# simplify23/TPS_PP

Hardware: NVIDIA B200
Metric: tps_pp_rectified_img_per_s (higher is better)
Workload: dtype f32

## Files before the change

### include/tpspp.h

```cpp
#ifndef TPSPP_H_
#define TPSPP_H_

#include <stddef.h>
#include <stdint.h>

#ifdef __cplusplus
extern "C" {
#endif

#define TPSPP_ABI_VERSION 2

#if defined(__GNUC__)
#define TPSPP_API __attribute__((visibility("default")))
#else
#define TPSPP_API
#endif

typedef struct CUstream_st* tpspp_stream_t;

enum {
  TPSPP_OK = 0,
  TPSPP_E_INVALID = -1,
  TPSPP_E_CUDA = -2,
  TPSPP_E_UNSUPPORTED = -3,
  TPSPP_E_NO_DEVICE = -4
};

enum { TPSPP_F32 = 0, TPSPP_BF16 = 1, TPSPP_SRC0_BF16 = 2 };

enum {
  TPSPP_MODE_ATTENTION = 0,
  TPSPP_MODE_CLASSICAL = 1
};

enum {
  TPSPP_VARIANT_AUTO = 0,
  TPSPP_VARIANT_GENERIC = 1,
  TPSPP_VARIANT_STAGED = 2,
  TPSPP_VARIANT_TILED = 3
};

typedef struct tpspp_warp_cfg {
  int32_t batch;
  int32_t channels0;
  int32_t src0_h, src0_w;
  int32_t channels1;
  int32_t src1_h, src1_w;
  int32_t out_h, out_w;
  int32_t num_fiducial;
  int32_t mode;
  float theta;
  int32_t feat_dtype;
  int32_t variant;
} tpspp_warp_cfg;

TPSPP_API int tpspp_version(void);
TPSPP_API const char* tpspp_last_error(void);

TPSPP_API int tpspp_device_info(int* sm_count, int* cc_major, int* cc_minor);

TPSPP_API int tpspp_launch_profile(int enable);
TPSPP_API int tpspp_launch_profile_read(float* ms, int capacity, int* count);

TPSPP_API size_t tpspp_warp_workspace_bytes(const tpspp_warp_cfg* cfg);

TPSPP_API size_t tpspp_warp_fwd_workspace_bytes(const tpspp_warp_cfg* cfg);

TPSPP_API int tpspp_warp_fwd(const tpspp_warp_cfg* cfg, const void* src0, const void* src1,
                   const float* c_prime, const float* pc_score, const float* P_hat,
                   const float* P, const float* inv_delta_C, void* out0, void* out1,
                   float* grid_out, void* workspace, tpspp_stream_t stream);

TPSPP_API int tpspp_sample_fwd(const tpspp_warp_cfg* cfg, const void* src0, const void* src1,
                     const float* grid, void* out0, void* out1, tpspp_stream_t stream);

TPSPP_API int tpspp_warp_bwd(const tpspp_warp_cfg* cfg, const void* src0, const void* src1,
                   const float* c_prime, const float* pc_score, const float* P_hat,
                   const float* P, const float* inv_delta_C, const void* gout0,
                   const void* gout1, void* gsrc0, void* gsrc1, float* g_c_prime,
                   float* g_pc_score, void* workspace, tpspp_stream_t stream);

enum {
  TPSPP_HEAD_FP32 = 0,
  TPSPP_HEAD_TC = 1,
  TPSPP_HEAD_BF16 = 2
};

typedef struct tpspp_head_cfg {
  int32_t batch;
  int32_t height, width;
  int32_t point_h, point_w;
  int32_t p_stride;
  int32_t precision;
  int32_t flags;
} tpspp_head_cfg;

enum { TPSPP_HEAD_FLAG_WEIGHTS_CACHED = 1, TPSPP_HEAD_FLAG_UNFUSED_DOWN = 2, TPSPP_HEAD_FLAG_UNFUSED_SCORE = 4,
       TPSPP_HEAD_FLAG_TF32X3_CONV = 8, TPSPP_HEAD_FLAG_FEATGRID_BF16 = 16 };

enum {
  TPSPP_P_ENC0_W = 0, TPSPP_P_ENC0_B, TPSPP_P_ENC1_W, TPSPP_P_ENC1_B, TPSPP_P_ENC2_W, TPSPP_P_ENC2_B,
  TPSPP_P_ENC3_W, TPSPP_P_ENC3_B, TPSPP_P_CBAM_MLP0_W, TPSPP_P_CBAM_MLP2_W, TPSPP_P_CBAM_SP_W,
  TPSPP_P_CBAM_SP_B, TPSPP_P_DEC0_W, TPSPP_P_DEC0_B, TPSPP_P_DEC1_W, TPSPP_P_DEC1_B, TPSPP_P_DEC2_W,
  TPSPP_P_DEC2_B, TPSPP_P_DEC3_W, TPSPP_P_DEC3_B, TPSPP_P_PLIN0_W, TPSPP_P_PLIN0_B, TPSPP_P_PLIN1_W,
  TPSPP_P_PLIN1_B, TPSPP_P_FLIN0_W, TPSPP_P_FLIN0_B, TPSPP_P_FLIN1_W, TPSPP_P_FLIN1_B,
  TPSPP_P_NORM1_W, TPSPP_P_NORM1_B, TPSPP_P_MLP_H_W, TPSPP_P_MLP_W_W, TPSPP_P_PROJ_W, TPSPP_P_PROJ_B,
  TPSPP_P_NORM2_W, TPSPP_P_NORM2_B, TPSPP_P_FC1_W, TPSPP_P_FC1_B, TPSPP_P_FC2_W, TPSPP_P_FC2_B,
  TPSPP_P_LOC1A_W, TPSPP_P_LOC1A_B, TPSPP_P_LOC1B_W, TPSPP_P_LOC1B_B, TPSPP_P_LOC2_W, TPSPP_P_LOC2_B,
  TPSPP_P_DOWN0_W, TPSPP_P_DOWN0_B, TPSPP_P_DOWN1_W, TPSPP_P_DOWN1_B, TPSPP_P_DOWN2_W, TPSPP_P_DOWN2_B,
  TPSPP_P_DOWN0_1_W, TPSPP_P_DOWN0_1_B, TPSPP_P_DOWN1_1_W, TPSPP_P_DOWN1_1_B, TPSPP_P_DOWNFEAT_W,
  TPSPP_P_DOWNFEAT_B, TPSPP_P_COUNT
};

enum {
  TPSPP_WS_F0 = 0, TPSPP_WS_F1, TPSPP_WS_F2, TPSPP_WS_A0, TPSPP_WS_A1, TPSPP_WS_E0, TPSPP_WS_E1,
  TPSPP_WS_E2, TPSPP_WS_E3 , TPSPP_WS_CBAM, TPSPP_WS_D0, TPSPP_WS_D1, TPSPP_WS_D2,
  TPSPP_WS_DE , TPSPP_WS_X1, TPSPP_WS_V, TPSPP_WS_DE2 ,
  TPSPP_WS_P1 ,
  TPSPP_WS_WPREP , TPSPP_WS_T1, TPSPP_WS_FS ,
  TPSPP_WS_HID , TPSPP_WS_P1IMG , TPSPP_WS_COUNT
};

TPSPP_API size_t tpspp_head_workspace_bytes(const tpspp_head_cfg* cfg);
TPSPP_API int tpspp_head_workspace_offsets(const tpspp_head_cfg* cfg, size_t* offsets);

TPSPP_API int tpspp_head_fwd(const tpspp_head_cfg* cfg, const float* x, const float* o0, const float* o1,
                             const float* const* params, float* feat_grid, float* c_prime,
                             float* pc_score, void* workspace, tpspp_stream_t stream);

typedef struct {
  int32_t batch;
  int32_t height, width;
  int32_t precision;
  int32_t flags;
} tpspp_stage_cfg;

enum {
  TPSPP_SP_CONV1_W = 0, TPSPP_SP_CONV1_B, TPSPP_SP_BN1_W, TPSPP_SP_BN1_B, TPSPP_SP_BN1_MEAN, TPSPP_SP_BN1_VAR,
  TPSPP_SP_LAYER1 = 6,
  TPSPP_SP_LAYER2 = 36,
  TPSPP_SP_COUNT = 81
};

TPSPP_API size_t tpspp_stage_workspace_bytes(const tpspp_stage_cfg* cfg);
TPSPP_API int tpspp_stage_fwd(const tpspp_stage_cfg* cfg, const float* img, const float* const* params, float* o0, float* o1,
                              float* x, void* workspace, tpspp_stream_t stream);

typedef struct {
  int32_t batch, channels;
  int32_t height, width;
  int32_t num_fiducial;
  int32_t flags;
} tpspp_locnet_cfg;
enum { TPSPP_LP_FC1_W = 20, TPSPP_LP_FC1_B, TPSPP_LP_FC2_W, TPSPP_LP_FC2_B, TPSPP_LP_COUNT = 24 };
TPSPP_API size_t tpspp_locnet_workspace_bytes(const tpspp_locnet_cfg* cfg);
TPSPP_API int tpspp_locnet_fwd(const tpspp_locnet_cfg* cfg, const float* img, const float* const* params, float* c_prime,
                               void* workspace, tpspp_stream_t stream);

typedef struct {
  int32_t batch, cin;
  int32_t height, width;
  int32_t ksize;
  int32_t stride_h, stride_w;
  int32_t relu;
  int32_t nsrc;
  int32_t up_h[3], up_w[3];
} tpspp_conv_cfg;
TPSPP_API size_t tpspp_conv_workspace_bytes(const tpspp_conv_cfg* cfg);
TPSPP_API int tpspp_conv_fwd(const tpspp_conv_cfg* cfg, const float* x, const float* w, const float* bias, float* y,
                             void* workspace, tpspp_stream_t stream);
TPSPP_API int tpspp_conv_bwd(const tpspp_conv_cfg* cfg, const float* x, const float* w, const float* y, const float* gy,
                             float* gx, float* gw, float* gb, void* workspace, tpspp_stream_t stream);

typedef struct {
  int64_t rows;
  int32_t in_features, out_features;
  int32_t weight_batches;
  int32_t flags;
} tpspp_linear_cfg;
enum { TPSPP_LINEAR_FLAG_WEIGHTS_CACHED = 1 };
TPSPP_API size_t tpspp_linear_workspace_bytes(const tpspp_linear_cfg* cfg);
// ... 54 lines not shown
```

### tps_pp_b200/_native.py

```python
from __future__ import annotations

import ctypes
import os
from ctypes import POINTER, Structure, c_char_p, c_float, c_int, c_int32, c_size_t, c_void_p

_HERE = os.path.dirname(os.path.abspath(__file__))
LIB_PATH = os.environ.get("TPSPP_LIB", os.path.join(_HERE, "libtpspp.so"))

OK = 0
F32, BF16, SRC0_BF16 = 0, 1, 2
MODE_ATTENTION, MODE_CLASSICAL = 0, 1
VARIANT_AUTO, VARIANT_GENERIC, VARIANT_STAGED, VARIANT_TILED = 0, 1, 2, 3


class WarpCfg(Structure):
    _fields_ = [
        ("batch", c_int32), ("channels0", c_int32), ("src0_h", c_int32), ("src0_w", c_int32),
        ("channels1", c_int32), ("src1_h", c_int32), ("src1_w", c_int32),
        ("out_h", c_int32), ("out_w", c_int32), ("num_fiducial", c_int32), ("mode", c_int32),
        ("theta", c_float), ("feat_dtype", c_int32), ("variant", c_int32),
    ]


class HeadCfg(Structure):
    _fields_ = [
        ("batch", c_int32), ("height", c_int32), ("width", c_int32), ("point_h", c_int32), ("point_w", c_int32),
        ("p_stride", c_int32), ("precision", c_int32), ("flags", c_int32),
    ]


class StageCfg(Structure):
    _fields_ = [("batch", c_int32), ("height", c_int32), ("width", c_int32), ("precision", c_int32), ("flags", c_int32)]


class ConvCfg(Structure):
    _fields_ = [("batch", c_int32), ("cin", c_int32), ("height", c_int32), ("width", c_int32), ("ksize", c_int32),
                ("stride_h", c_int32), ("stride_w", c_int32), ("relu", c_int32), ("nsrc", c_int32),
                ("up_h", c_int32 * 3), ("up_w", c_int32 * 3)]


class LocnetCfg(Structure):
    _fields_ = [("batch", c_int32), ("channels", c_int32), ("height", c_int32), ("width", c_int32), ("num_fiducial", c_int32),
                ("flags", c_int32)]


LP_COUNT = 24


class AttnCfg(Structure):
    _fields_ = [("batch", c_int32), ("heads", c_int32), ("head_dim", c_int32), ("kv_len", c_int32), ("kv_capacity", c_int32),
                ("temperature", c_float), ("q_stride", c_int32), ("new_stride", c_int32), ("kv_head_major", c_int32)]


class AttnEncodeCfg(Structure):
    _fields_ = [("batch", c_int32), ("heads", c_int32), ("head_dim", c_int32), ("seq_len", c_int32), ("temperature", c_float),
                ("row_stride", c_int32)]


class OcrPrepCfg(Structure):
    _fields_ = [("n", c_int32), ("out_h", c_int32), ("out_w", c_int32), ("mean", c_float * 3), ("std", c_float * 3),
                ("pad_value", c_int32), ("flags", c_int32), ("packed_bytes", ctypes.c_int64)]


class LinearCfg(Structure):
    _fields_ = [("rows", ctypes.c_int64), ("in_features", c_int32), ("out_features", c_int32), ("weight_batches", c_int32),
                ("flags", c_int32)]


SP_COUNT = 81
HEAD_FP32, HEAD_TC, HEAD_BF16 = 0, 1, 2
HEAD_FLAG_WEIGHTS_CACHED = 1
HEAD_FLAG_UNFUSED_DOWN = 2
HEAD_FLAG_UNFUSED_SCORE = 4
HEAD_FLAG_TF32X3_CONV = 8
HEAD_FLAG_FEATGRID_BF16 = 16
LINEAR_FLAG_WEIGHTS_CACHED = 1
ACT_NONE, ACT_GELU = 0, 1
ABI_VERSION = 2
P_COUNT = 58
WS_NAMES = ("f0", "f1", "f2", "a0", "a1", "e0", "e1", "e2", "e3", "cbam", "d0", "d1", "d2", "de", "x1", "v", "de2", "p1", "wprep", "t1", "fs", "hid", "p1img")

_SIGNATURES = {
    "tpspp_version": (c_int, []),
    "tpspp_last_error": (c_char_p, []),
    "tpspp_last_launch_count": (c_int, []),
    "tpspp_launch_profile": (c_int, [c_int]),
    "tpspp_launch_profile_read": (c_int, [POINTER(ctypes.c_float), c_int, POINTER(c_int)]),
    "tpspp_device_info": (c_int, [POINTER(c_int), POINTER(c_int), POINTER(c_int)]),
    "tpspp_warp_workspace_bytes": (c_size_t, [POINTER(WarpCfg)]),
    "tpspp_warp_fwd_workspace_bytes": (c_size_t, [POINTER(WarpCfg)]),
    "tpspp_warp_fwd": (c_int, [POINTER(WarpCfg)] + [c_void_p] * 12),
    "tpspp_sample_fwd": (c_int, [POINTER(WarpCfg)] + [c_void_p] * 6),
    "tpspp_warp_bwd": (c_int, [POINTER(WarpCfg)] + [c_void_p] * 15),
    "tpspp_head_workspace_bytes": (c_size_t, [POINTER(HeadCfg)]),
    "tpspp_head_workspace_offsets": (c_int, [POINTER(HeadCfg), POINTER(c_size_t)]),
    "tpspp_head_fwd": (c_int, [POINTER(HeadCfg), c_void_p, c_void_p, c_void_p, POINTER(c_void_p),
                               c_void_p, c_void_p, c_void_p, c_void_p, c_void_p]),
    "tpspp_conv_workspace_bytes": (c_size_t, [POINTER(ConvCfg)]),
    "tpspp_conv_fwd": (c_int, [POINTER(ConvCfg)] + [c_void_p] * 6),
    "tpspp_conv_bwd": (c_int, [POINTER(ConvCfg)] + [c_void_p] * 9),
    "tpspp_convcat_fwd": (c_int, [POINTER(ConvCfg), POINTER(c_void_p)] + [c_void_p] * 5),
    "tpspp_convcat_bwd": (c_int, [POINTER(ConvCfg), POINTER(c_void_p)] + [c_void_p] * 3 + [POINTER(c_void_p)] + [c_void_p] * 4),
    "tpspp_locnet_workspace_bytes": (c_size_t, [POINTER(LocnetCfg)]),
    "tpspp_locnet_fwd": (c_int, [POINTER(LocnetCfg), c_void_p, POINTER(c_void_p), c_void_p, c_void_p, c_void_p]),
    "tpspp_attn_decode": (c_int, [POINTER(AttnCfg)] + [c_void_p] * 8),
    "tpspp_attn_encode": (c_int, [POINTER(AttnEncodeCfg)] + [c_void_p] * 6),
    "tpspp_ocr_prep": (c_int, [POINTER(OcrPrepCfg)] + [c_void_p] * 4),
    "tpspp_linear_fwd_ex": (c_int, [POINTER(LinearCfg)] + [c_void_p] * 4 + [c_int32] + [c_void_p] * 3),
    "tpspp_linear_ln_fwd": (c_int, [POINTER(LinearCfg)] + [c_void_p] * 4 + [c_int32] + [c_void_p] * 3 + [ctypes.c_float] + [c_void_p] * 3),
    "tpspp_linear_workspace_bytes": (c_size_t, [POINTER(LinearCfg)]),
    "tpspp_linear_fwd": (c_int, [POINTER(LinearCfg)] + [c_void_p] * 6),
    "tpspp_linear_bwd": (c_int, [POINTER(LinearCfg)] + [c_void_p] * 8),
    "tpspp_stage_workspace_bytes": (c_size_t, [POINTER(StageCfg)]),
    "tpspp_stage_fwd": (c_int, [POINTER(StageCfg), c_void_p, POINTER(c_void_p), c_void_p, c_void_p, c_void_p, c_void_p,
                                c_void_p]),
}
_OPTIONAL = {}

_lib = None


def exported_symbols():
    return sorted(_SIGNATURES)


def lib() -> ctypes.CDLL:
    global _lib
    if _lib is None:
        if not os.path.exists(LIB_PATH):
            raise RuntimeError(
                f"libtpspp.so not found at {LIB_PATH}: build it with `python -m tps_pp_b200.build` "
                "(there is no CPU/PyTorch fallback for the TPS++ hot path)")
        handle = ctypes.CDLL(LIB_PATH)
        for name, (res, args) in {**_SIGNATURES, **_OPTIONAL}.items():
            try:
                fn = getattr(handle, name)
            except AttributeError:
                if name in _OPTIONAL:
                    continue
                raise RuntimeError(f"{LIB_PATH} does not export {name}; rebuild it")
            fn.restype = res
            fn.argtypes = args
        if handle.tpspp_version() != ABI_VERSION:
            raise RuntimeError("libtpspp ABI version mismatch; rebuild it")
        _lib = handle
    return _lib


def last_error() -> str:
    return lib().tpspp_last_error().decode("utf-8", "replace")


def check(rc: int, what: str) -> None:
    if rc != OK:
        raise RuntimeError(f"{what} failed (code {rc}): {last_error()}")


def last_launch_count() -> int:
# ... 8 lines not shown
```

### tps_pp_b200/backbone.py

```python
from __future__ import annotations

from typing import Optional, Sequence

import torch
import torch.nn as nn
import torch.nn.functional as F

from . import functional as TF
from .registry import BACKBONES


class BasicBlock(nn.Module):
    expansion = 1

    def __init__(self, inplanes, planes, stride=1, downsample=None):
        super().__init__()
        self.conv1 = nn.Conv2d(inplanes, planes, kernel_size=1, stride=1, bias=False)
        self.bn1 = nn.BatchNorm2d(planes)
        self.relu = nn.ReLU(inplace=True)
        self.conv2 = nn.Conv2d(planes, planes, kernel_size=3, stride=stride, padding=1, bias=False)
        self.bn2 = nn.BatchNorm2d(planes)
        self.downsample = downsample
        self.stride = stride

    def forward(self, x):
        out = self.relu(self.bn1(self.conv1(x)))
        out = self.bn2(self.conv2(out))
        identity = x if self.downsample is None else self.downsample(x)
        return self.relu(out + identity)


@BACKBONES.register_module()
class ResNetABI_v2_large(nn.Module):
    def __init__(self, in_channels=3, stem_channels=32, base_channels=32, arch_settings=[3, 4, 6, 6, 3],
                 strides=[2, 1, 2, 1, 1], p_strides=[2, 1, 2, 1, 1], out_indices=None, last_stage_pool=False,
                 init_cfg=[dict(type='Xavier', layer='Conv2d'), dict(type='Constant', val=1, layer='BatchNorm2d')]):
        super().__init__()
        assert isinstance(in_channels, int)
        assert isinstance(stem_channels, int)
        assert isinstance(arch_settings, list) and all(isinstance(v, int) for v in arch_settings)
        assert isinstance(strides, list) and all(isinstance(v, int) for v in strides)
        assert len(arch_settings) == len(strides)
        assert out_indices is None or isinstance(out_indices, (list, tuple))
        assert isinstance(last_stage_pool, bool)
        self.init_cfg = init_cfg
        self.out_indices = out_indices
        self.last_stage_pool = last_stage_pool
        self.arch_settings = list(arch_settings)
        self.strides = list(strides)
        self.in_channels, self.stem_channels, self.base_channels = in_channels, stem_channels, base_channels
        self.conv1 = nn.Conv2d(in_channels, stem_channels, kernel_size=3, stride=1, padding=1)
        self.bn1 = nn.BatchNorm2d(stem_channels)
        self.relu1 = nn.ReLU()
        self.res_layers = []
        inplanes, planes = stem_channels, base_channels
        for i, blocks in enumerate(arch_settings):
            stride = strides[i]
            downsample = None
            if stride != 1 or inplanes != planes:
                downsample = nn.Sequential(nn.Conv2d(inplanes, planes, 1, stride, bias=False), nn.BatchNorm2d(planes))
            layers = [BasicBlock(inplanes, planes, stride=stride, downsample=downsample)]
            layers += [BasicBlock(planes, planes) for _ in range(1, blocks)]
            name = f'layer{i + 1}'
            self.add_module(name, nn.Sequential(*layers))
            self.res_layers.append(name)
            inplanes = planes
            planes *= 2
        self.stage_impl = "auto"
        self._stage_ws = {}
        self._last_stage_native = None

    def init_weights(self):
        for m in self.modules():
            if isinstance(m, nn.Conv2d):
                nn.init.xavier_normal_(m.weight, gain=1)
                if m.bias is not None:
                    nn.init.constant_(m.bias, 0)
            elif isinstance(m, nn.BatchNorm2d):
                nn.init.constant_(m.weight, 1)
                nn.init.constant_(m.bias, 0)

    def _stage_native_ok(self, x) -> bool:
        if self.stage_impl == "library":
            return False
        ok = (x.is_cuda and x.dtype == torch.float32 and x.dim() == 4 and x.shape[1] == 3 and x.shape[3] == 128
              and x.shape[2] % 4 == 0 and not self.training and not torch.is_grad_enabled()
              and self.in_channels == 3 and self.stem_channels == 32 and self.base_channels == 32
              and self.arch_settings[:2] == [3, 4] and self.strides[:2] == [1, 2])
        if self.stage_impl == "native" and not ok:
            raise RuntimeError("tps_pp_b200: stage_impl='native' needs eval mode, torch.no_grad(), fp32 CUDA images "
                               "[B,3,4k,128] and the nrtr_tps++ geometry (arch_settings[:2]=[3,4], strides[:2]=[1,2])")
        return ok

    def stage_tensors(self):
        out = [self.conv1.weight, self.conv1.bias, self.bn1.weight, self.bn1.bias, self.bn1.running_mean, self.bn1.running_var]
        for layer in (self.layer1, self.layer2):
            for blk in layer:
                out += [blk.conv1.weight, blk.bn1.weight, blk.bn1.bias, blk.bn1.running_mean, blk.bn1.running_var,
                        blk.conv2.weight, blk.bn2.weight, blk.bn2.bias, blk.bn2.running_mean, blk.bn2.running_var]
                if blk.downsample is not None:
                    ds = blk.downsample
                    out += [ds[0].weight, ds[1].weight, ds[1].bias, ds[1].running_mean, ds[1].running_var]
        return out

    def stage(self, img: torch.Tensor):
        self._last_stage_native = self._stage_native_ok(img)
        if self._last_stage_native:
            tensors = self.stage_tensors()
            key = (img.device.index, torch.cuda.current_stream(img.device).cuda_stream)
            stamp = (img.shape[0], img.shape[2], tuple((t.data_ptr(), t._version) for t in tensors))
            ws, ws_stamp = self._stage_ws.get(key, (None, None))
            o0, o1, x, ws = TF.stage_forward(img, tensors, ws, weights_cached=(ws_stamp == stamp))
            if len(self._stage_ws) >= 8 and key not in self._stage_ws:
                self._stage_ws.clear()
            self._stage_ws[key] = (ws, stamp)
            return x, [o0, o1]
        if not img.is_cuda:
            raise RuntimeError("tps_pp_b200.ResNetABI_v2_large runs on CUDA tensors only; there is no CPU fallback")
        x = self.relu1(self.bn1(self.conv1(img)))
        outs = []
        for name in self.res_layers[:2]:
            outs.append(x)
            x = getattr(self, name)(x)
        return x, outs

    def forward(self, x, tpsnet=None, test=False, **kwargs):
        x, outs = self.stage(x)
        outputs = None
        for i, name in enumerate(self.res_layers):
            if i < 2:
                continue
            if i == 2 and tpsnet is not None:
                outputs = tpsnet(x, outs, **kwargs)
                if outputs.get('output', None) is not None:
                    x = outputs['output']
            outs.append(x)
            x = getattr(self, name)(x)
        return {'output': x, 'img_ref': outputs.get('output', None) if outputs is not None else None}

    def return_feature(self, x, tpsnet=None, test=False):
        x, outs = self.stage(x)
        if tpsnet is None:
            return x
        for name in self.res_layers[2:]:
            x = getattr(self, name)(x)
        return x
```

### tps_pp_b200/csrc/common.cuh

```cuda
#pragma once
#include <cuda_runtime.h>
#include <cuda_bf16.h>
#include <stdint.h>
#include <stdio.h>
#include <stdarg.h>

#include "../../include/tpspp.h"

#if defined(__CUDA_ARCH__) && (__CUDA_ARCH__ < 1000)
#error "libtpspp is written for sm_100a (B200) only"
#endif

namespace tpspp {

void set_error(const char* fmt, ...);
void count_launch(int n = 1);
void prof_begin(cudaStream_t st);
void reset_launch_count();
int sm_count();
bool pdl_on();
void pdl_scope(bool on);
template <typename... KArgs, typename... Args>
inline void launch_k(void (*kern)(KArgs...), dim3 grid, dim3 block, size_t smem, cudaStream_t st, Args&&... args) {
  cudaLaunchConfig_t cfg = {};
  cfg.gridDim = grid;
  cfg.blockDim = block;
  cfg.dynamicSmemBytes = smem;
  cfg.stream = st;
  cudaLaunchAttribute at[1];
  at[0].id = cudaLaunchAttributeProgrammaticStreamSerialization;
  at[0].val.programmaticStreamSerializationAllowed = 1;
  cfg.attrs = at;
  cfg.numAttrs = pdl_on() ? 1 : 0;
  if (cudaLaunchKernelEx(&cfg, kern, static_cast<KArgs>(args)...) != cudaSuccess && cfg.numAttrs != 0) {
    cudaGetLastError();
    cfg.numAttrs = 0;
    cudaLaunchKernelEx(&cfg, kern, static_cast<KArgs>(args)...);
  }
}
#ifdef __CUDACC__
__device__ __forceinline__ void pdl_wait() { asm volatile("griddepcontrol.wait;" ::: "memory"); }
__device__ __forceinline__ void pdl_trigger() { asm volatile("griddepcontrol.launch_dependents;" ::: "memory"); }
#endif

#define TPSPP_CHECK_CUDA(expr)                                                        \
  do {                                                                                \
    cudaError_t _e = (expr);                                                          \
    if (_e != cudaSuccess) {                                                          \
      tpspp::set_error("%s failed: %s (%s:%d)", #expr, cudaGetErrorString(_e),        \
                       __FILE__, __LINE__);                                           \
      return TPSPP_E_CUDA;                                                            \
    }                                                                                 \
  } while (0)

#define TPSPP_REQUIRE(cond, ...)                                                      \
  do {                                                                                \
    if (!(cond)) {                                                                    \
      tpspp::set_error(__VA_ARGS__);                                                  \
      return TPSPP_E_INVALID;                                                         \
    }                                                                                 \
  } while (0)

struct WarpParams {
  int B, C0, H0, W0, C1, H1, W1, n, F, K;
  int mode;
  float theta;
  const void* src0;
  const void* src1;
  const float* c_prime;
  const float* score;
  const float* P_hat;
  const float* P;
  const float* hatC;
  const float* grid_in;
  void* out0;
  void* out1;
  float* grid_out;
  const void* gout0;
  const void* gout1;
  void* gsrc0;
  void* gsrc1;
  double* T_ws;
  float* g_grid;
  float* g_c_prime;
  float* g_score;
};

int validate_cfg(const tpspp_warp_cfg* cfg);
void fill_params(const tpspp_warp_cfg* cfg, WarpParams* p);
int bwd_nsplit(const tpspp_warp_cfg* cfg);

#ifdef __CUDACC__

struct Taps {
  int off, dx, dy;
  float w[4];
};

template <typename CT>
__device__ __forceinline__ CT clip_coord(CT v, int size) {
  return fmin((CT)(size - 1), fmax(v, (CT)0));
}

template <typename CT>
__device__ __forceinline__ Taps make_taps(CT gx, CT gy, int W, int H) {
  CT ix = ((gx + (CT)1) / (CT)2) * (CT)(W - 1);
  CT iy = ((gy + (CT)1) / (CT)2) * (CT)(H - 1);
  ix = clip_coord<CT>(ix, W);
  iy = clip_coord<CT>(iy, H);
  CT x0f = floor(ix), y0f = floor(iy);
  int x0 = (int)x0f, y0 = (int)y0f;
  CT tx = ix - x0f, ty = iy - y0f;
  CT ux = (x0f + (CT)1) - ix, uy = (y0f + (CT)1) - iy;
  Taps t;
  t.off = y0 * W + x0;
  t.dx = (x0 + 1 < W) ? 1 : 0;
  t.dy = (y0 + 1 < H) ? W : 0;
  t.w[0] = (float)(ux * uy);
  t.w[1] = t.dx ? (float)(tx * uy) : 0.f;
  t.w[2] = t.dy ? (float)(ux * ty) : 0.f;
  t.w[3] = (t.dx && t.dy) ? (float)(tx * ty) : 0.f;
// ... 205 lines not shown
```

### tps_pp_b200/csrc/head.cu

```cuda
#include "head.cuh"

#include <string.h>

namespace tpspp {

constexpr int CV_TM = 128;
constexpr int CV_KC = 32;
constexpr int CV_WLD = 68;
constexpr int CV_SMEM = (2 * CV_KC * CV_TM + 2 * CV_KC * CV_WLD) * 4;

template <int KS>
__global__ void __launch_bounds__(256, 2) conv_ffma_kernel(ConvArgs a) {
  extern __shared__ __align__(16) float smem[];
  float* As = smem;
  float* Ws = smem + 2 * CV_KC * CV_TM;
  constexpr int TAPS = KS * KS;
  const int tid = threadIdx.x;
  const int HoWo = a.Ho * a.Wo;
  const long long Mtot = (long long)a.B * HoWo;
  const long long m_base = (long long)blockIdx.x * CV_TM;
  const int Ktot = a.Ctot * TAPS;
  const int nchunks = (Ktot + CV_KC - 1) / CV_KC;

  const int lp = tid & (CV_TM - 1), lk0 = tid >> 7;
// ... 720 lines not shown
    }
#pragma unroll
    for (int i = 0; i < 8; ++i) {
      const int px = p0 + (i < 4 ? tx * 4 + i : 64 + tx * 4 + (i - 4));
      if (px >= n) continue;
      float* o = a.score + ((size_t)b * n + px) * F;
      const int k = ty * 2;
      if (k < F) o[k] = tanhf(acc[i][0] * a.scale);
      if (k + 1 < F) o[k + 1] = tanhf(acc[i][1] * a.scale);
    }
  }
}

struct HeadDims {
  int B, h, w, H2, W2, F, py, px, ps;
  int h1, w1, h2, w2;
};

static int head_dims(const tpspp_head_cfg* c, HeadDims* d) {
  TPSPP_REQUIRE(c != nullptr, "head cfg is NULL");
  TPSPP_REQUIRE(c->batch >= 0, "batch must be >= 0");
  TPSPP_REQUIRE(c->width == 64, "TPS_PP head needs feature-map width 64 (DGAB linear layers act on the width axis; "
                                "reference DGAB.py:36,52 -- SURVEY F4), got %d", c->width);
  TPSPP_REQUIRE(c->height >= 8 && c->height <= DG_MAXH && c->height % 8 == 0, "height must be a multiple of 8 in [8,%d]", DG_MAXH);
  TPSPP_REQUIRE(c->p_stride == 1 || c->p_stride == 2, "p_stride must be 1 or 2");
  d->B = c->batch; d->h = c->height; d->w = c->width; d->H2 = 2 * c->height; d->W2 = 2 * c->width;
  d->ps = c->p_stride;
  d->h1 = d->h / 2; d->w1 = d->w / 2;
  d->h2 = d->h1 / d->ps; d->w2 = d->w1 / d->ps;
  d->py = d->h2 / 2; d->px = d->w2;
  d->F = d->py * d->px;
  TPSPP_REQUIRE(d->py == c->point_h && d->px == c->point_w,
                "point_size (%d,%d) must equal the MSFA encoder's output lattice (%d,%d) (SURVEY F4)", c->point_h,
                c->point_w, d->py, d->px);
  TPSPP_REQUIRE(d->F <= 32 && d->F % 2 == 0, "num_fiducial must be even and <= 32 for the score kernel (got %d)", d->F);
  TPSPP_REQUIRE(c->precision == TPSPP_HEAD_FP32 || c->precision == TPSPP_HEAD_TC || c->precision == TPSPP_HEAD_BF16,
                "unknown precision %d", c->precision);
  return TPSPP_OK;
}

struct ConvLayerDesc { int w_idx, Ctot, KS, N, NT; };
constexpr int kNumTcLayers = 18;
enum { TCL_FLIN0 = 14, TCL_FLIN1 = 15, TCL_FC1 = 16, TCL_FC2 = 17 };
static const ConvLayerDesc kConvLayers[kNumTcLayers] = {
    {TPSPP_P_DOWN0_W, 32, 1, 64, 64},   {TPSPP_P_DOWN1_W, 32, 1, 64, 64},    {TPSPP_P_DOWN2_W, 64, 1, 64, 64},
    {TPSPP_P_DOWN0_1_W, 64, 3, 64, 64}, {TPSPP_P_DOWN1_1_W, 64, 3, 64, 64},  {TPSPP_P_DOWNFEAT_W, 192, 1, 64, 64},
    {TPSPP_P_ENC0_W, 192, 3, 64, 64},   {TPSPP_P_ENC1_W, 64, 3, 64, 64},     {TPSPP_P_ENC2_W, 64, 3, 64, 64},
    {TPSPP_P_ENC3_W, 64, 3, 64, 64},    {TPSPP_P_DEC0_W, 64, 3, 64, 64},     {TPSPP_P_DEC1_W, 64, 3, 64, 64},
    {TPSPP_P_DEC2_W, 64, 3, 64, 64},    {TPSPP_P_DEC3_W, 64, 3, 64, 64},
    {TPSPP_P_FLIN0_W, 64, 1, 32, 32},   {TPSPP_P_FLIN1_W, 32, 1, 128, 64},   {TPSPP_P_FC1_W, 64, 1, 256, 64},
    {TPSPP_P_FC2_W, 256, 1, 64, 64}};
static size_t wprep_total_floats() {
  size_t t = 0;
  for (int i = 0; i < kNumTcLayers; ++i) t += conv_tc_wprep_floats(kConvLayers[i].Ctot, kConvLayers[i].KS, kConvLayers[i].N);
  return t;
}

static void head_offsets(const HeadDims& d, size_t* off, size_t* total) {
  const size_t B = d.B;
  size_t sz[TPSPP_WS_COUNT];
  const size_t big = B * 64 * d.H2 * d.W2, mid = B * 64 * d.h * d.w;
  sz[TPSPP_WS_F0] = big; sz[TPSPP_WS_F1] = big; sz[TPSPP_WS_F2] = mid; sz[TPSPP_WS_A0] = mid; sz[TPSPP_WS_A1] = mid;
  sz[TPSPP_WS_E0] = mid; sz[TPSPP_WS_E1] = B * 64 * d.h1 * d.w1; sz[TPSPP_WS_E2] = B * 64 * d.h2 * d.w2;
  sz[TPSPP_WS_E3] = B * 64 * d.F; sz[TPSPP_WS_CBAM] = B * 64 * d.F; sz[TPSPP_WS_D0] = sz[TPSPP_WS_E2];
  sz[TPSPP_WS_D1] = sz[TPSPP_WS_E1]; sz[TPSPP_WS_D2] = mid; sz[TPSPP_WS_DE] = mid; sz[TPSPP_WS_X1] = mid;
  sz[TPSPP_WS_V] = mid; sz[TPSPP_WS_DE2] = mid; sz[TPSPP_WS_P1] = B * d.F * 128;
  sz[TPSPP_WS_WPREP] = wprep_total_floats();
  sz[TPSPP_WS_T1] = B * d.h * d.w * 32;
  sz[TPSPP_WS_FS] = B * d.h * d.w * 128;
  sz[TPSPP_WS_HID] = mid * 4;
  sz[TPSPP_WS_P1IMG] = B * 8192;
  size_t cur = 0;
  for (int i = 0; i < TPSPP_WS_COUNT; ++i) {
    off[i] = cur;
    cur += (sz[i] * sizeof(float) + 255) / 256 * 256;
  }
  *total = cur + 256;
}

static ConvSrc mk_src(const float* p, int C, int H, int W, int nhwc, int uh = 1, int uw = 1, int bf16 = 0) {
  ConvSrc s; s.ptr = p; s.C = C; s.H = H; s.W = W; s.uh = uh; s.uw = uw; s.nhwc = nhwc; s.bf16 = bf16; return s;
}

static int run_conv(int KS, ConvSrc s0, ConvSrc s1, ConvSrc s2, const float* w, const float* bias, const float* skip,
                    float* out, int out_nhwc, int B, int Ho, int Wo, int sh, int sw, cudaStream_t st,
                    const float* wprep = nullptr, int mode = CM_TF32X3, int out_bf16 = 0, int skip_bf16 = 0) {
  ConvArgs a;
  a.out_nhwc = out_nhwc; a.out_bf16 = out_bf16; a.skip_bf16 = skip_bf16;
  a.act = CONV_ACT_RELU; a.act_scale = 1.f; a.Cout = 64; a.wimg_stride = 0; a.skip_pre = 0; a.out_cstride = 0; a.zi = 0;
  a.src[0] = s0; a.src[1] = s1; a.src[2] = s2;
  a.weight = w; a.bias = bias; a.skip = skip; a.out = out;
  a.B = B; a.Ho = Ho; a.Wo = Wo; a.Ctot = s0.C + s1.C + s2.C; a.sh = sh; a.sw = sw; a.pad = (KS == 3) ? 1 : 0;
  if (wprep != nullptr && conv_tc_eligible(a, KS)) return run_conv_tc(KS, a, wprep, 64, st, mode);
  const long long M = (long long)B * Ho * Wo;
  const unsigned grid = (unsigned)((M + CV_TM - 1) / CV_TM);
  if (KS == 1) conv_ffma_kernel<1><<<grid, 256, CV_SMEM, st>>>(a);
  else conv_ffma_kernel<3><<<grid, 256, CV_SMEM, st>>>(a);
  count_launch();
  TPSPP_CHECK_CUDA(cudaGetLastError());
  return TPSPP_OK;
}

static int head_attrs_once() {
  static thread_local int done_dev = -1;
  int dev = 0;
  TPSPP_CHECK_CUDA(cudaGetDevice(&dev));
  if (done_dev == dev) return TPSPP_OK;
  TPSPP_CHECK_CUDA(cudaFuncSetAttribute(conv_ffma_kernel<1>, cudaFuncAttributeMaxDynamicSharedMemorySize, CV_SMEM));
  TPSPP_CHECK_CUDA(cudaFuncSetAttribute(conv_ffma_kernel<3>, cudaFuncAttributeMaxDynamicSharedMemorySize, CV_SMEM));
  TPSPP_CHECK_CUDA(cudaFuncSetAttribute(dgab_mlp_kernel, cudaFuncAttributeMaxDynamicSharedMemorySize, ML_SMEM));
  TPSPP_CHECK_CUDA(cudaFuncSetAttribute(score_kernel, cudaFuncAttributeMaxDynamicSharedMemorySize, SC_SMEM));
  TPSPP_CHECK_CUDA(cudaFuncSetAttribute(loc_p1_kernel, cudaFuncAttributeMaxDynamicSharedMemorySize, 64 * 1024));
  done_dev = dev;
  return TPSPP_OK;
}

}

using namespace tpspp;

extern "C" size_t tpspp_head_workspace_bytes(const tpspp_head_cfg* cfg) {
  HeadDims d;
  if (head_dims(cfg, &d) != TPSPP_OK) return 0;
  size_t off[TPSPP_WS_COUNT], total;
  head_offsets(d, off, &total);
  return total;
}

extern "C" int tpspp_head_workspace_offsets(const tpspp_head_cfg* cfg, size_t* offsets) {
  HeadDims d;
  int rc = head_dims(cfg, &d);
  if (rc != TPSPP_OK) return rc;
  TPSPP_REQUIRE(offsets != nullptr, "offsets is NULL");
  size_t total;
  head_offsets(d, offsets, &total);
  return TPSPP_OK;
}

extern "C" int tpspp_head_fwd(const tpspp_head_cfg* cfg, const float* x, const float* o0, const float* o1,
                              const float* const* P, float* feat_grid, float* c_prime, float* pc_score,
                              void* workspace, tpspp_stream_t stream) {
  reset_launch_count();
  prof_begin((cudaStream_t)stream);
  HeadDims d;
  int rc = head_dims(cfg, &d);
  if (rc != TPSPP_OK) return rc;
  if (d.B == 0) return TPSPP_OK;
  TPSPP_REQUIRE(x && o0 && o1 && P && feat_grid && c_prime && pc_score && workspace, "tpspp_head_fwd: null pointer");
  TPSPP_REQUIRE(((uintptr_t)workspace & 255) == 0, "tpspp_head_fwd: workspace must be 256-byte aligned");
  for (int i = 0; i < TPSPP_P_COUNT; ++i) {
    TPSPP_REQUIRE(P[i] != nullptr, "tpspp_head_fwd: params[%d] is NULL", i);
    TPSPP_REQUIRE(((uintptr_t)P[i] & 15) == 0, "tpspp_head_fwd: params[%d] must be 16-byte aligned (vector loads)", i);
  }
  if (d.B == 0) return TPSPP_OK;
  rc = head_attrs_once();
  if (rc != TPSPP_OK) return rc;
  cudaStream_t st = (cudaStream_t)stream;
  struct PdlScope { PdlScope(bool on) { pdl_scope(on); } ~PdlScope() { pdl_scope(false); } } pdl_guard(cfg->precision != TPSPP_HEAD_FP32);
  size_t off[TPSPP_WS_COUNT], total;
  head_offsets(d, off, &total);
  auto W = [&](int i) { return reinterpret_cast<float*>((char*)workspace + off[i]); };
  const ConvSrc none = mk_src(nullptr, 0, 1, 1, 0);
  constexpr int NCHW = 0, NHWC = 1;
  const int B = d.B, h = d.h, w = d.w, H2 = d.H2, W2 = d.W2;

  const float* wp[kNumTcLayers];
  for (int i = 0; i < kNumTcLayers; ++i) wp[i] = nullptr;
  const bool bf16 = cfg->precision == TPSPP_HEAD_BF16;
  const bool tc = cfg->precision == TPSPP_HEAD_TC || bf16;
  const bool weights_cached = (cfg->flags & TPSPP_HEAD_FLAG_WEIGHTS_CACHED) != 0;
  int cmode[14];
  for (int i = 0; i < 14; ++i) {
    const bool one = kConvLayers[i].KS == 1;
    cmode[i] = (bf16 && !one) ? CM_BF16 : ((one || (cfg->flags & TPSPP_HEAD_FLAG_TF32X3_CONV)) ? CM_TF32X3 : CM_MIX);
  }
  if (tc) {
    WPrepLayer L[kNumTcLayers];
    float* cur = W(TPSPP_WS_WPREP);
    for (int i = 0; i < kNumTcLayers; ++i) {
      L[i].w = P[kConvLayers[i].w_idx]; L[i].out = cur; L[i].Ctot = kConvLayers[i].Ctot;
      L[i].taps = kConvLayers[i].KS * kConvLayers[i].KS; L[i].N = kConvLayers[i].N; L[i].NT = kConvLayers[i].NT; L[i].scale = nullptr; L[i].dg_cin = 0; L[i].dg_ci0 = 0;
      L[i].bf16 = i < 14 ? cmode[i] : CM_TF32X3;
      wp[i] = cur;
      cur += conv_tc_wprep_floats(kConvLayers[i].Ctot, kConvLayers[i].KS, kConvLayers[i].N);
    }
    if (!weights_cached) {
      rc = conv_tc_prepare_weights(L, kNumTcLayers, st);
      if (rc != TPSPP_OK) return rc;
    }
  }
#define RUN(...) do { rc = run_conv(__VA_ARGS__); if (rc != TPSPP_OK) return rc; } while (0)
  bool fused_down = false;
  if (tc && !(cfg->flags & TPSPP_HEAD_FLAG_UNFUSED_DOWN)) {
    rc = run_down_fused(x, o0, o1, wp[0], wp[1], wp[2], wp[5], P[TPSPP_P_DOWN0_B], P[TPSPP_P_DOWN1_B], P[TPSPP_P_DOWN2_B],
                        P[TPSPP_P_DOWNFEAT_B], W(TPSPP_WS_F0), W(TPSPP_WS_F1), W(TPSPP_WS_F2), feat_grid, B, h, w, st, bf16 ? 1 : 0,
                        (bf16 && (cfg->flags & TPSPP_HEAD_FLAG_FEATGRID_BF16)) ? 1 : 0);
    if (rc < 0) return rc;
    fused_down = rc == TPSPP_OK;
    TPSPP_REQUIRE(fused_down || !bf16, "head: the bf16 mode needs the fused down kernel's geometry (width 64, 16-byte aligned inputs)");
  }
  const int bs = (bf16 && fused_down) ? 1 : 0;
  if (!fused_down) {
  RUN(1, mk_src(o0, 32, H2, W2, NCHW), none, none, P[TPSPP_P_DOWN0_W], P[TPSPP_P_DOWN0_B], nullptr, W(TPSPP_WS_F0), NCHW, B, H2, W2, 1, 1, st, wp[0], cmode[0]);
  RUN(1, mk_src(o1, 32, H2, W2, NCHW), none, none, P[TPSPP_P_DOWN1_W], P[TPSPP_P_DOWN1_B], nullptr, W(TPSPP_WS_F1), NCHW, B, H2, W2, 1, 1, st, wp[1], cmode[1]);
  RUN(1, mk_src(x, 64, h, w, NCHW), none, none, P[TPSPP_P_DOWN2_W], P[TPSPP_P_DOWN2_B], nullptr, W(TPSPP_WS_F2), NCHW, B, h, w, 1, 1, st, wp[2], cmode[2]);
  }
  RUN(3, mk_src(W(TPSPP_WS_F0), 64, H2, W2, NCHW, 1, 1, bs), none, none, P[TPSPP_P_DOWN0_1_W], P[TPSPP_P_DOWN0_1_B], nullptr, W(TPSPP_WS_A0), NCHW, B, h, w, 2, 2, st, wp[3], cmode[3], bs);
  RUN(3, mk_src(W(TPSPP_WS_F1), 64, H2, W2, NCHW, 1, 1, bs), none, none, P[TPSPP_P_DOWN1_1_W], P[TPSPP_P_DOWN1_1_B], nullptr, W(TPSPP_WS_A1), NCHW, B, h, w, 2, 2, st, wp[4], cmode[4], bs);
  if (!fused_down)
  RUN(1, mk_src(W(TPSPP_WS_F0), 64, H2, W2, NCHW), mk_src(W(TPSPP_WS_F1), 64, H2, W2, NCHW), mk_src(W(TPSPP_WS_F2), 64, h, w, NCHW, 2, 2),
      P[TPSPP_P_DOWNFEAT_W], P[TPSPP_P_DOWNFEAT_B], nullptr, feat_grid, NCHW, B, H2, W2, 1, 1, st, wp[5], cmode[5]);
  RUN(3, mk_src(W(TPSPP_WS_A0), 64, h, w, NCHW, 1, 1, bs), mk_src(W(TPSPP_WS_A1), 64, h, w, NCHW, 1, 1, bs), mk_src(W(TPSPP_WS_F2), 64, h, w, NCHW, 1, 1, bs),
      P[TPSPP_P_ENC0_W], P[TPSPP_P_ENC0_B], nullptr, W(TPSPP_WS_E0), NCHW, B, h, w, 1, 1, st, wp[6], cmode[6], bs);
  RUN(3, mk_src(W(TPSPP_WS_E0), 64, h, w, NCHW, 1, 1, bs), none, none, P[TPSPP_P_ENC1_W], P[TPSPP_P_ENC1_B], nullptr, W(TPSPP_WS_E1), NCHW, B, d.h1, d.w1, 2, 2, st, wp[7], cmode[7]);
  RUN(3, mk_src(W(TPSPP_WS_E1), 64, d.h1, d.w1, NCHW), none, none, P[TPSPP_P_ENC2_W], P[TPSPP_P_ENC2_B], nullptr, W(TPSPP_WS_E2), NCHW, B, d.h2, d.w2, d.ps, d.ps, st, wp[8], cmode[8]);
  RUN(3, mk_src(W(TPSPP_WS_E2), 64, d.h2, d.w2, NCHW), none, none, P[TPSPP_P_ENC3_W], P[TPSPP_P_ENC3_B], nullptr, W(TPSPP_WS_E3), NCHW, B, d.py, d.px, 2, 1, st, wp[9], cmode[9]);
  launch_k(cbam_kernel, dim3(B), dim3(256), 0, st, (const float*)W(TPSPP_WS_E3), W(TPSPP_WS_CBAM), P[TPSPP_P_CBAM_MLP0_W], P[TPSPP_P_CBAM_MLP2_W],
           P[TPSPP_P_CBAM_SP_W], P[TPSPP_P_CBAM_SP_B], d.py, d.px);
  count_launch();
  TPSPP_CHECK_CUDA(cudaGetLastError());
  RUN(3, mk_src(W(TPSPP_WS_CBAM), 64, d.py, d.px, NCHW, 2, 1), none, none, P[TPSPP_P_DEC0_W], P[TPSPP_P_DEC0_B], W(TPSPP_WS_E2), W(TPSPP_WS_D0), NCHW, B, d.h2, d.w2, 1, 1, st, wp[10], cmode[10]);
  RUN(3, mk_src(W(TPSPP_WS_D0), 64, d.h2, d.w2, NCHW, d.ps, d.ps), none, none, P[TPSPP_P_DEC1_W], P[TPSPP_P_DEC1_B], W(TPSPP_WS_E1), W(TPSPP_WS_D1), NCHW, B, d.h1, d.w1, 1, 1, st, wp[11], cmode[11]);
  RUN(3, mk_src(W(TPSPP_WS_D1), 64, d.h1, d.w1, NCHW, 2, 2), none, none, P[TPSPP_P_DEC2_W], P[TPSPP_P_DEC2_B], W(TPSPP_WS_E0), W(TPSPP_WS_D2), NCHW, B, h, w, 1, 1, st, wp[12], cmode[12], bs, bs);
  RUN(3, mk_src(W(TPSPP_WS_D2), 64, h, w, NCHW, 1, 1, bs), none, none, P[TPSPP_P_DEC3_W], P[TPSPP_P_DEC3_B], nullptr, W(TPSPP_WS_DE), NCHW, B, h, w, 1, 1, st, wp[13], cmode[13]);
#undef RUN
  {
    LocArgs a;
    a.e3 = W(TPSPP_WS_E3);
    a.wa = P[TPSPP_P_LOC1A_W]; a.ba = P[TPSPP_P_LOC1A_B]; a.wb = P[TPSPP_P_LOC1B_W]; a.bb = P[TPSPP_P_LOC1B_B];
    a.wc = P[TPSPP_P_LOC2_W]; a.bc = P[TPSPP_P_LOC2_B];
    a.wp0 = P[TPSPP_P_PLIN0_W]; a.bp0 = P[TPSPP_P_PLIN0_B]; a.wp1 = P[TPSPP_P_PLIN1_W]; a.bp1 = P[TPSPP_P_PLIN1_B];
    a.c_prime = c_prime; a.p1 = W(TPSPP_WS_P1); a.F = d.F;
    a.p1img = (tc && d.F == 32) ? W(TPSPP_WS_P1IMG) : nullptr;
    const size_t smem = (size_t)(d.F * 65 + d.F * 256 + 2 * d.F + d.F * 33) * sizeof(float);
    launch_k(loc_p1_kernel, dim3(B), dim3(256), smem, st, a);
    count_launch();
    TPSPP_CHECK_CUDA(cudaGetLastError());
  }
  {
    DgabArgs a;
    a.x = W(TPSPP_WS_DE); a.e3 = W(TPSPP_WS_E3);
    a.n1w = P[TPSPP_P_NORM1_W]; a.n1b = P[TPSPP_P_NORM1_B]; a.n2w = P[TPSPP_P_NORM2_W]; a.n2b = P[TPSPP_P_NORM2_B];
    a.wh = P[TPSPP_P_MLP_H_W]; a.ww = P[TPSPP_P_MLP_W_W]; a.wp = P[TPSPP_P_PROJ_W]; a.bp = P[TPSPP_P_PROJ_B];
    a.x1 = W(TPSPP_WS_X1); a.v = W(TPSPP_WS_V); a.H = h; a.F = d.F;
    {
      TPSPP_REQUIRE((h == 8 || h == 16) && d.F <= 32 && dgab_warp_smem(h, d.F) <= 220 * 1024, "DGAB: unsupported geometry h=%d F=%d", h, d.F);
      const size_t smem = dgab_warp_smem(h, d.F);
      auto kern = h == 8 ? dgab_warp_kernel<8> : dgab_warp_kernel<16>;
      TPSPP_CHECK_CUDA(cudaFuncSetAttribute(kern, cudaFuncAttributeMaxDynamicSharedMemorySize, (int)smem));
      int grid = sm_count();
      if (grid > (B * 64 + DW_WARPS - 1) / DW_WARPS) grid = (B * 64 + DW_WARPS - 1) / DW_WARPS;
      launch_k(kern, dim3(grid), dim3(DW_WARPS * 32), smem, st, a, B * 64);
    }
    count_launch();
    TPSPP_CHECK_CUDA(cudaGetLastError());
    const long long R = (long long)B * 64 * h;
    if (tc) {
      rc = run_mlp_fused(W(TPSPP_WS_V), W(TPSPP_WS_X1), wp[TCL_FC1], P[TPSPP_P_FC1_B], wp[TCL_FC2], P[TPSPP_P_FC2_B],
                         W(TPSPP_WS_DE2), R, st);
      if (rc < 0) return rc;
      if (rc == 1) {
      ConvArgs g;
      memset(&g, 0, sizeof(g));
      g.src[0] = mk_src(W(TPSPP_WS_V), 64, 1, (int)R, NHWC); g.src[1] = none; g.src[2] = none;
      g.B = 1; g.Ho = 1; g.Wo = (int)R; g.Ctot = 64; g.sh = 1; g.sw = 1; g.pad = 0; g.out_nhwc = 1;
      g.bias = P[TPSPP_P_FC1_B]; g.skip = nullptr; g.out = W(TPSPP_WS_HID); g.act = CONV_ACT_GELU; g.act_scale = 1.f;
      g.Cout = 256; g.wimg_stride = 0; g.weight = nullptr;
      rc = run_conv_tc(1, g, wp[TCL_FC1], 64, st);
      if (rc != TPSPP_OK) return rc;
      g.src[0] = mk_src(W(TPSPP_WS_HID), 256, 1, (int)R, NHWC); g.Ctot = 256;
      g.bias = P[TPSPP_P_FC2_B]; g.skip = W(TPSPP_WS_X1); g.out = W(TPSPP_WS_DE2); g.act = CONV_ACT_NONE; g.Cout = 64;
      rc = run_conv_tc(1, g, wp[TCL_FC2], 64, st);
      if (rc != TPSPP_OK) return rc;
      }
// ... 50 lines not shown
```

### tps_pp_b200/csrc/head.cuh

```cuda
#pragma once
#include "common.cuh"

namespace tpspp {

struct ConvSrc {
  const float* ptr;
  int C, H, W, uh, uw;
  int nhwc;
  int bf16;
};
struct ConvArgs {
  ConvSrc src[3];
  const float* weight;
  const float* bias;
  const float* skip;
  float* out;
  int B, Ho, Wo, Ctot, sh, sw, pad;
  int out_nhwc;
  int act;
  float act_scale;
  int Cout;
  long long wimg_stride;
  int skip_pre;
  int out_cstride;
  int zi;
  int out_bf16, skip_bf16;
  int splitk;
};
enum { CONV_ACT_RELU = 0, CONV_ACT_NONE = 1, CONV_ACT_GELU = 2, CONV_ACT_TANH = 3 };
enum { CM_TF32X3 = 0, CM_BF16 = 1, CM_MIX = 2 };


bool conv_tc_eligible(const ConvArgs& a, int KS);
int run_conv_tc(int KS, const ConvArgs& a, const float* wprep, int NT, cudaStream_t st, int mode = CM_TF32X3);
int run_mlp_fused(const float* v, const float* x1, const float* w1img, const float* b1, const float* w2img, const float* b2,
                  float* out, long long R, cudaStream_t st);
int run_down_fused(const float* x, const float* o0, const float* o1, const float* w0img, const float* w1img, const float* w2img,
                   const float* wfimg, const float* b0, const float* b1, const float* b2, const float* bf, float* f0, float* f1,
                   float* f2, float* fg, int B, int h, int w, cudaStream_t st, int out_bf16 = 0, int fg_bf16 = 0);
int run_score_fused(const float* de2, const float* w0img, const float* w1img, const float* p1img, const float* b0, const float* b1,
                    float* score, int B, int h, int w, int F, float scale, cudaStream_t st);
size_t conv_tc_wprep_floats(int Ctot, int KS, int N);

struct WPrepLayer {
  const float* w;
  float* out;
  int Ctot, taps, N, NT;
  const float* scale;
  int dg_cin, dg_ci0;
  int bf16;
};
constexpr int WPREP_MAX_LAYERS = 20;
size_t wgrad_rows_ws_floats(long long R, int K, int N, int batches);
int run_wgrad_rows(const float* gy, const float* x, float* gw, float* gb, long long R, int K, int N, int batches, float* ws,
                   cudaStream_t st);
int conv_tc_prepare_weights(const WPrepLayer* layers, int nlayers, cudaStream_t st);

}
```

### tps_pp_b200/csrc/head_tc.cu

```cuda
#include "head.cuh"
#include "tc.cuh"

#include <cuda.h>
#include <string.h>

namespace tpspp {

constexpr int TC_TM = 128, TC_KC = 32;
constexpr int TC_A_LBO = TC_TM * 16 + 16;
constexpr int TC_A_BYTES = (TC_KC / 4) * TC_A_LBO;
__host__ __device__ constexpr int tc_b_bytes(int NT) { return NT * TC_KC * 4; }
__host__ __device__ constexpr int tc_stage_bytes(int NT) { return 2 * TC_A_BYTES + 2 * tc_b_bytes(NT); }
__host__ __device__ constexpr int tc_smem_bytes(int NT) { return 2 * tc_stage_bytes(NT) + 64 + TC_TM * 16; }
constexpr int TC_PRODUCERS = 256, TC_THREADS = TC_PRODUCERS + 32;
__host__ __device__ constexpr int tc_tmem_cols(int NT) { return NT == 64 ? 256 : 128; }

struct ConvTcArgs {
  ConvArgs c;
  const float* wprep;
};

__device__ __forceinline__ float tc_gelu(float x) { return 0.5f * x * (1.f + erff(x * 0.70710678118654752440f)); }
__device__ __forceinline__ float tc_gelu_fast(float x) {
  const float z = fabsf(x) * 0.70710678118654752440f;
// ... 161 lines not shown
      if (lane == 0) mbar_arrive(&fbars[buf]);
    };
    gather(va);
    if (nchunks > 1) gather(vb);
    for (int ch = 0; ch < nchunks; ch += 2) {
      produce(ch, va);
      if (ch + 1 < nchunks) produce(ch + 1, vb);
    }
    const int last = nchunks - 1;
    mbar_wait_bounded(&bars[last & 1], (uint32_t)((last >> 1) & 1));
    tc_fence_after();
  }
  if (warp < TC_PRODUCERS / 32) {
    const int wq = warp & 3, half = warp >> 2;
    const long long m = m_base + wq * 32 + lane;
    const int b = (m < Mtot) ? (int)(m / HoWo) : 0;
    const int rem = (m < Mtot) ? (int)(m - (long long)b * HoWo) : 0;
#pragma unroll 1
    for (int pass = 0; pass < HC / 16; ++pass) {
      float acc[16], part[16];
      const uint32_t taddr = tmem_d + ((uint32_t)(wq * 32) << 16) + (uint32_t)(half * HC + pass * 16);
      tmem_ld_cols<16>(taddr, acc);
      tmem_ld_cols<16>(taddr + 2 * NT, part);
#pragma unroll
      for (int j = 0; j < 16; ++j) acc[j] += part[j];
      if (nchunks > 1) {
        tmem_ld_cols<16>(taddr + NT, part);
#pragma unroll
        for (int j = 0; j < 16; ++j) acc[j] += part[j];
      }
      const int cb = co_off + half * HC + pass * 16;
      if (m < Mtot && a.out_nhwc) {
        const size_t o0 = (size_t)m * a.Cout + cb;
#pragma unroll
        for (int j = 0; j < 16; j += 4) {
          float4 bs = make_float4(0.f, 0.f, 0.f, 0.f);
          if (a.bias != nullptr) bs = __ldg(reinterpret_cast<const float4*>(a.bias + cb + j));
          float4 r = make_float4(tc_act(acc[j] + bs.x, a.act, a.act_scale), tc_act(acc[j + 1] + bs.y, a.act, a.act_scale),
                                 tc_act(acc[j + 2] + bs.z, a.act, a.act_scale), tc_act(acc[j + 3] + bs.w, a.act, a.act_scale));
          if (a.skip != nullptr) {
            const float4 sk = __ldg(reinterpret_cast<const float4*>(a.skip + o0 + j));
            r.x += sk.x; r.y += sk.y; r.z += sk.z; r.w += sk.w;
          }
          *reinterpret_cast<float4*>(a.out + o0 + j) = r;
        }
      } else if (m < Mtot) {
        const size_t o0 = ((size_t)b * a.Cout + cb) * HoWo + rem;
#pragma unroll
        for (int j = 0; j < 16; ++j) {
          float r = tc_act(acc[j] + (a.bias != nullptr ? __ldg(a.bias + cb + j) : 0.f), a.act, a.act_scale);
          const size_t o = o0 + (size_t)j * HoWo;
          if (a.skip != nullptr) r += __ldg(a.skip + o);
          a.out[o] = r;
        }
      }
    }
  }
  tc_fence_before();
  __syncthreads();
  if (warp == 0) tmem_dealloc(tmem_d, tc_tmem_cols(NT));
}


__host__ __device__ constexpr uint32_t mix_b_bf(int NT) { return (uint32_t)NT * 128u; }
__host__ __device__ constexpr uint32_t mix_b_lo(int NT) { return (uint32_t)NT * 192u; }
constexpr uint32_t MIX_B_BF = mix_b_bf(64), MIX_B_LO = mix_b_lo(64);

template <int NT>
__device__ __forceinline__ void mix_mma_chunk(uint32_t tmem_d, uint32_t a_base, uint32_t b_base, uint32_t idesc_tf, uint32_t idesc_bf,
                                              bool first) {
#pragma unroll
  for (int j = 0; j < TC_KC / 16; ++j) {
    const uint64_t dbw = umma_smem_desc(b_base + mix_b_bf(NT) + j * 2 * (NT * 16), NT * 16, 128);
    const uint64_t dbl = umma_smem_desc(b_base + mix_b_lo(NT) + j * 2 * (NT * 16), NT * 16, 128);
    umma_ts_f16(tmem_d + 64, a_base + 32 + j * 8, dbw, idesc_bf, (first && j == 0) ? 0u : 1u);
    umma_ts_f16(tmem_d + 64, a_base + 48 + j * 8, dbl, idesc_bf, 1u);
  }
#pragma unroll
  for (int j = 0; j < TC_KC / 8; ++j) {
    const uint64_t dbh = umma_smem_desc(b_base + j * 2 * (NT * 16), NT * 16, 128);
    umma_ts_tf32(tmem_d, a_base + j * 8, dbh, idesc_tf, (first && j == 0) ? 0u : 1u);
  }
}
template <int NT>
__device__ __forceinline__ void mix_mma_chunk_probed(uint32_t d, uint32_t a_base, uint64_t bdesc0, uint32_t idesc_tf, uint32_t idesc_bf,
                                                     uint32_t accumulate, uint32_t commit_bar, uint32_t next_a_bar, uint32_t next_w_bar,
                                                     uint32_t next_parity, uint32_t& ok_a, uint32_t& ok_w) {
  constexpr int KS2 = 2 * NT, BW0 = 8 * NT, BL0 = 12 * NT;
  asm volatile(
      "{\n"
      ".reg .pred pa, pw, pf, pt;\n"
      ".reg .b64 dsc;\n"
      ".reg .b32 ta, tc;\n"
      "mbarrier.test_wait.parity.shared::cta.b64 pa, [%2], %4;\n"
      "mbarrier.test_wait.parity.shared::cta.b64 pw, [%3], %4;\n"
      "setp.ne.b32 pf, %9, 0;\n"
      "setp.eq.u32 pt, %4, %4;\n"
      "add.u32 tc, %5, 64;\n"
      "add.u32 ta, %6, 32;\n add.u64 dsc, %7, %12;\n"
      "tcgen05.mma.cta_group::1.kind::f16 [tc], [ta], dsc, %11, pf;\n"
      "add.u32 ta, %6, 48;\n add.u64 dsc, %7, %13;\n"
      "tcgen05.mma.cta_group::1.kind::f16 [tc], [ta], dsc, %11, pt;\n"
      "add.u32 ta, %6, 40;\n add.u64 dsc, %7, %14;\n"
      "tcgen05.mma.cta_group::1.kind::f16 [tc], [ta], dsc, %11, pt;\n"
      "add.u32 ta, %6, 56;\n add.u64 dsc, %7, %15;\n"
      "tcgen05.mma.cta_group::1.kind::f16 [tc], [ta], dsc, %11, pt;\n"
      "tcgen05.mma.cta_group::1.kind::tf32 [%5], [%6], %7, %10, pf;\n"
      "add.u32 ta, %6, 8;\n add.u64 dsc, %7, %16;\n"
      "tcgen05.mma.cta_group::1.kind::tf32 [%5], [ta], dsc, %10, pt;\n"
      "add.u32 ta, %6, 16;\n add.u64 dsc, %7, %17;\n"
      "tcgen05.mma.cta_group::1.kind::tf32 [%5], [ta], dsc, %10, pt;\n"
      "add.u32 ta, %6, 24;\n add.u64 dsc, %7, %18;\n"
      "tcgen05.mma.cta_group::1.kind::tf32 [%5], [ta], dsc, %10, pt;\n"
      "tcgen05.commit.cta_group::1.mbarrier::arrive::one.shared::cluster.b64 [%8];\n"
      "selp.u32 %0, 1, 0, pa;\n"
      "selp.u32 %1, 1, 0, pw;\n"
      "}\n"
      : "=r"(ok_a), "=r"(ok_w)
      : "r"(next_a_bar), "r"(next_w_bar), "r"(next_parity), "r"(d), "r"(a_base), "l"(bdesc0), "r"(commit_bar), "r"(accumulate),
        "r"(idesc_tf), "r"(idesc_bf), "n"(BW0), "n"(BL0), "n"(BW0 + KS2), "n"(BL0 + KS2), "n"(KS2), "n"(2 * KS2), "n"(3 * KS2)
      : "memory");
}
__device__ __forceinline__ void mix_split(const float (&v)[16], float (&hi)[16], uint32_t (&lo2)[8], uint32_t (&a2)[8]) {
#pragma unroll
  for (int i = 0; i < 16; ++i) hi[i] = __uint_as_float(__float_as_uint(v[i]) & 0xFFFFE000u);
#pragma unroll
  for (int i = 0; i < 8; ++i) {
    const __nv_bfloat162 l2 = __floats2bfloat162_rn(v[2 * i] - hi[2 * i], v[2 * i + 1] - hi[2 * i + 1]);
    const __nv_bfloat162 x2 = __floats2bfloat162_rn(v[2 * i], v[2 * i + 1]);
    lo2[i] = *reinterpret_cast<const uint32_t*>(&l2);
    a2[i] = *reinterpret_cast<const uint32_t*>(&x2);
  }
}
__device__ __forceinline__ void mix_store_a(uint32_t stage_addr, int kh, const float (&v)[16]) {
  float hi[16];
  uint32_t lo2[8], a2[8];
#pragma unroll
  for (int i = 0; i < 16; ++i) hi[i] = __uint_as_float(__float_as_uint(v[i]) & 0xFFFFE000u);
#pragma unroll
  for (int i = 0; i < 8; ++i) {
    const __nv_bfloat162 l2 = __floats2bfloat162_rn(v[2 * i] - hi[2 * i], v[2 * i + 1] - hi[2 * i + 1]);
    const __nv_bfloat162 x2 = __floats2bfloat162_rn(v[2 * i], v[2 * i + 1]);
    lo2[i] = *reinterpret_cast<const uint32_t*>(&l2);
    a2[i] = *reinterpret_cast<const uint32_t*>(&x2);
  }
  tmem_st16(stage_addr + (uint32_t)(kh * 16), hi);
  tmem_st8(stage_addr + (uint32_t)(32 + kh * 8), lo2);
  tmem_st8(stage_addr + (uint32_t)(48 + kh * 8), a2);
}

template <int PLANE>
__device__ __forceinline__ void ts_load16(const float* q, float (&v)[16], bool ok) {
#pragma unroll
  for (int i = 0; i < 16; ++i) v[i] = ok ? __ldg(q + i * PLANE) : 0.f;
}

constexpr int TS_B_BYTES = tc_b_bytes(64);
constexpr int TS_STAGE = 2 * TS_B_BYTES;
constexpr int TS_SMEM = 2 * TS_STAGE + 64 + TC_TM * 16 + 256;

template <int KS, int MODE>
__global__ void __launch_bounds__(TC_THREADS, 2) conv_ts_kernel(ConvTcArgs t) {
  constexpr bool BF16 = MODE == CM_BF16, MIX = MODE == CM_MIX;
  constexpr int NT = 64;
  constexpr int W_BYTES = BF16 ? NT * TC_KC * 2 : 2 * TS_B_BYTES;
  constexpr int A_COL0 = BF16 ? 64 : 128;
  constexpr int A_STAGE = BF16 ? 16 : 64;
  constexpr int TMEM_COLS = BF16 ? 128 : 256;
  extern __shared__ __align__(1024) unsigned char smem[];
  uint64_t* bars = reinterpret_cast<uint64_t*>(smem + 2 * TS_STAGE);
  uint64_t* wbars = bars + 2;
  uint64_t* fbars = bars + 4;
  uint32_t* tmem_slot = reinterpret_cast<uint32_t*>(bars + 6);
  int4* geo = reinterpret_cast<int4*>(smem + 2 * TS_STAGE + 64);
  float* bias_s = reinterpret_cast<float*>(smem + 2 * TS_STAGE + 64 + TC_TM * 16);
  const ConvArgs& a = t.c;
  const int tid = threadIdx.x, lane = tid & 31;
  const int warp = __shfl_sync(0xffffffffu, tid >> 5, 0);

  if (tid == 0) {
    mbar_init(&bars[0], 1); mbar_init(&bars[1], 1);
    mbar_init(&wbars[0], 1); mbar_init(&wbars[1], 1);
    mbar_init(&fbars[0], TC_PRODUCERS / 32); mbar_init(&fbars[1], TC_PRODUCERS / 32);
    fence_barrier_init();
  }
  if (tid < NT) bias_s[tid] = (a.bias != nullptr && tid < a.Cout) ? __ldg(a.bias + tid) : 0.f;
  if (warp == 0) tmem_alloc(tmem_slot, TMEM_COLS);
  tc_fence_before();
  __syncthreads();
  tc_fence_after();
  const uint32_t tmem_d = *tmem_slot;
  pdl_trigger();
  pdl_wait();

  const int HoWo = a.Ho * a.Wo;
  const long long Mtot = (long long)a.B * HoWo;
  const long long m_base = (long long)blockIdx.x * TC_TM;
  const int Ctot = a.Ctot;
  const int nchunks = (Ctot * KS * KS) / TC_KC;
  const unsigned char* wimg = reinterpret_cast<const unsigned char*>(t.wprep);

  if (tid < TC_TM) {
    const long long lm = m_base + tid;
    int4 gq = make_int4(0, 0, 0, 0);
    if (lm < Mtot) {
// ... 125 lines not shown
      tc_fence_before();
      __syncwarp();
      if (lane == 0) mbar_arrive(&fbars[buf]);
    };
    gather(va);
    if (nchunks > 1) gather(vb);
    for (int ch = 0; ch < nchunks; ch += 2) {
      produce(ch, va);
      if (ch + 1 < nchunks) produce(ch + 1, vb);
    }
    const int last = nchunks - 1;
    mbar_wait_bounded(&bars[last & 1], (uint32_t)((last >> 1) & 1));
    tc_fence_after();

    const int wq = warp & 3, half = warp >> 2;
    const long long m = m_base + wq * 32 + lane;
    const int b = (m < Mtot) ? (int)(m / HoWo) : 0;
    const int rem = (m < Mtot) ? (int)(m - (long long)b * HoWo) : 0;
#pragma unroll 1
    for (int pass = 0; pass < 2; ++pass) {
      float acc[16], part[16];
      const uint32_t taddr = lane_addr + (uint32_t)(half * 32 + pass * 16);
      tmem_ld_cols<16>(taddr, acc);
      if (!BF16) {
        tmem_ld_cols<16>(taddr + 64, part);
#pragma unroll
        for (int j = 0; j < 16; ++j) acc[j] += part[j];
      }
      const int cb = half * 32 + pass * 16;
      if (m < Mtot && a.out_nhwc) {
        const size_t o0 = (size_t)m * a.Cout + cb;
#pragma unroll
        for (int j = 0; j < 16; j += 4) {
          float4 bs = make_float4(0.f, 0.f, 0.f, 0.f);
          if (a.bias != nullptr) bs = __ldg(reinterpret_cast<const float4*>(a.bias + cb + j));
          float4 r = make_float4(tc_act(acc[j] + bs.x, a.act, a.act_scale), tc_act(acc[j + 1] + bs.y, a.act, a.act_scale),
                                 tc_act(acc[j + 2] + bs.z, a.act, a.act_scale), tc_act(acc[j + 3] + bs.w, a.act, a.act_scale));
          if (a.skip != nullptr) {
            const float4 sk = __ldg(reinterpret_cast<const float4*>(a.skip + o0 + j));
            r.x += sk.x; r.y += sk.y; r.z += sk.z; r.w += sk.w;
          }
          *reinterpret_cast<float4*>(a.out + o0 + j) = r;
        }
      } else if (m < Mtot) {
        const float4* b4 = reinterpret_cast<const float4*>(bias_s + cb);
#pragma unroll
        for (int j = 0; j < 16; j += 4) {
          const float4 bs = b4[j >> 2];
          acc[j] += bs.x; acc[j + 1] += bs.y; acc[j + 2] += bs.z; acc[j + 3] += bs.w;
        }
        const size_t o0 = ((size_t)b * (a.out_cstride ? a.out_cstride : a.Cout) + cb) * HoWo + rem;
        if (cb >= a.Cout) continue;
        if (a.skip != nullptr && a.skip_pre) {
          const float* sk = a.skip + o0;
#pragma unroll
          for (int j = 0; j < 16; ++j) acc[j] += __ldg(sk + (size_t)j * HoWo);
        }
        if (a.act == CONV_ACT_RELU) {
#pragma unroll
          for (int j = 0; j < 16; ++j) acc[j] = fmaxf(acc[j], 0.f);
        } else {
#pragma unroll
          for (int j = 0; j < 16; ++j) acc[j] = tc_act(acc[j], a.act, a.act_scale);
        }
        if (a.skip != nullptr && !a.skip_pre) {
          const float* sk = a.skip + o0;
#pragma unroll
          for (int j = 0; j < 16; ++j) acc[j] += __ldg(sk + (size_t)j * HoWo);
        }
        float* po = a.out + o0;
#pragma unroll
        for (int j = 0; j < 16; ++j) po[(size_t)j * HoWo] = acc[j];
      }
    }
  }
  tc_fence_before();
  __syncthreads();
  if (warp == 0) tmem_dealloc(tmem_d, TMEM_COLS);
}

struct ConvTmaArgs {
  ConvTcArgs t;
  CUtensorMap tmap[3];
  int TW, TH, BW, BH;
  int TX, TPI;
  int S;
  int XH;
};
constexpr int TM_XH = 4;
constexpr int TM_TILE_MAX = 32 * (4 * 72) * 4;
constexpr int TM_TILE_BF = 17408;
__host__ __device__ constexpr int tm_tile_bytes(int KS) { return KS == 3 ? ((TM_TILE_MAX + 1023) / 1024) * 1024 : 16384; }
__host__ __device__ constexpr int tm_tile_bufs(int KS) { return KS == 3 ? 2 : 4; }
__host__ __device__ constexpr int tm_smem_bytes(int KS) { return tm_tile_bufs(KS) * tm_tile_bytes(KS) + 2 * TS_STAGE + (KS == 3 ? 4096 : 0) + 512 + 1024; }
constexpr int TM_THREADS = TC_THREADS + 32;

__device__ __forceinline__ void tma_load_4d(void* dst, const CUtensorMap* tm, int c0, int c1, int c2, int c3, uint64_t* bar,
                                            uint64_t policy) {
  asm volatile(
      "cp.async.bulk.tensor.4d.shared::cluster.global.mbarrier::complete_tx::bytes.L2::cache_hint "
      "[%0], [%1, {%3, %4, %5, %6}], [%2], %7;" ::"r"(smem_u32(dst)),
      "l"(reinterpret_cast<uint64_t>(tm)), "r"(smem_u32(bar)), "r"(c0), "r"(c1), "r"(c2), "r"(c3), "l"(policy)
      : "memory");
}

template <int KS, int MODE, int NT = 64>
__global__ void __launch_bounds__(TM_THREADS, 2) conv_tma_kernel(const __grid_constant__ ConvTmaArgs g) {
  constexpr bool BF16 = MODE == CM_BF16, MIX = MODE == CM_MIX;
  constexpr int T = KS * KS;
  static_assert(NT == 64 || NT == 32, "64 or 32 output channels per tile");
  const int XH = g.XH;
  const bool SBF = (BF16 && KS == 3) && g.t.c.src[0].bf16 != 0;
  const int ntb_rt = SBF ? 4 : tm_tile_bufs(KS);
  const int tile_stride = SBF ? TM_TILE_BF : tm_tile_bytes(KS);
  constexpr int CT = (BF16 && KS == 3) ? 3 : 1;
  constexpr int W_TAP = BF16 ? NT * TC_KC * 2 : 2 * tc_b_bytes(NT);
  constexpr int W_BYTES = CT * W_TAP;
  constexpr int NS = (BF16 && KS == 3) ? 3 : 2;
  constexpr int A_BASE = NS == 3 ? 64 : 128, A_STRIDE = NS == 3 ? 48 : 64;
  constexpr int WS_STRIDE = NS == 3 ? 12288 : TS_STAGE;
  constexpr int TILE_BYTES = tm_tile_bytes(KS);
  constexpr int NTB = tm_tile_bufs(KS);
  extern __shared__ unsigned char smem_raw[];
  unsigned char* smem = reinterpret_cast<unsigned char*>((reinterpret_cast<uintptr_t>(smem_raw) + 1023) & ~(uintptr_t)1023);
  unsigned char* tiles = smem;
  unsigned char* wst = smem + NTB * TILE_BYTES;
  uint64_t* bars = reinterpret_cast<uint64_t*>(wst + (NS == 3 ? 3 * 12288 : 2 * TS_STAGE));
  uint64_t* a_empty = bars;
  uint64_t* a_full = bars + 3;
  uint64_t* w_full = bars + 6;
  uint64_t* t_full = bars + 9;
  uint64_t* t_empty = bars + 13;
  uint64_t* d_empty = bars + 17;
  uint32_t* tmem_slot = reinterpret_cast<uint32_t*>(bars + 18);
  float* bias_s = reinterpret_cast<float*>(bars + 20);
  const ConvArgs& a = g.t.c;
  const int tid = threadIdx.x, lane = tid & 31;
  const int warp = __shfl_sync(0xffffffffu, tid >> 5, 0);

  if (tid == 0) {
    for (int i = 0; i < NS; ++i) { mbar_init(&a_empty[i], 1); mbar_init(&a_full[i], TC_PRODUCERS / 32); mbar_init(&w_full[i], 1); }
    for (int i = 0; i < 4; ++i) { mbar_init(&t_full[i], 1); mbar_init(&t_empty[i], TC_PRODUCERS / 32); }
    mbar_init(d_empty, TC_PRODUCERS / 32);
    fence_barrier_init();
  }
  if (tid < NT) bias_s[tid] = (a.bias != nullptr && tid < a.Cout) ? __ldg(a.bias + tid) : 0.f;
  if (warp == 0) tmem_alloc(tmem_slot, 256);
  tc_fence_before();
  __syncthreads();
  tc_fence_after();
  const uint32_t tmem_d = *tmem_slot;
  pdl_trigger();
  pdl_wait();

  const int HoWo = a.Ho * a.Wo;
  const int ntiles = (int)(((long long)a.B * HoWo) / TC_TM);
  const int ncc = a.Ctot / TC_KC;
  const int nchunks = ncc * T / CT;
  const int CHS = g.BW * g.BH;
  const uint32_t tile_tx = (uint32_t)(CHS * TC_KC * (SBF ? 2 : 4));
  const unsigned char* wimg = reinterpret_cast<const unsigned char*>(g.t.wprep);
  constexpr uint32_t IDESC = umma_instr_desc(TC_TM, NT, BF16 ? 1 : 2);
  constexpr uint32_t IDESC_BF = umma_instr_desc(TC_TM, NT, 1);

  const int S = g.S, NG = (KS == 3 && S == 2) ? 3 : 1, TG = T / NG;
  auto issue_tile = [&](int tile, int cc, int grp, int gcc) {
    const int img = tile / g.TPI;
    const int trem = tile - img * g.TPI;
    const int tyy = trem / g.TX;
    const int oy0 = tyy * g.TH, ox0 = (trem - tyy * g.TX) * g.TW;
    int s = 0, c0 = cc * TC_KC;
    if (c0 >= a.src[0].C) { c0 -= a.src[0].C; s = 1; if (c0 >= a.src[1].C) { c0 -= a.src[1].C; s = 2; } }
    const int up = (s == 0 ? a.src[0].uh : (s == 1 ? a.src[1].uh : a.src[2].uh)) == 2;
    const int y0 = S * oy0 - a.pad + grp;
    const int tb = gcc % ntb_rt;
    mbar_arrive_expect_tx(&t_full[tb], tile_tx);
    if (SBF)
      tma_load_4d(tiles + tb * tile_stride, &g.tmap[s], c0, S * ox0 - XH, y0, img, &t_full[tb], policy_evict_first());
    else
      tma_load_4d(tiles + tb * tile_stride, &g.tmap[s], up ? ((ox0 - 2 * XH) >> 1) : (S * ox0 - XH), up ? (y0 >> 1) : y0, c0, img,
                  &t_full[tb], policy_evict_first());
  };

  if (warp == TC_PRODUCERS / 32) {
    int gch = 0, it = 0;
    int ok_a = 0, ok_w = 0;
    for (int tile = blockIdx.x; tile < ntiles; tile += gridDim.x, ++it) {
      if (it >= 1) {
        mbar_wait_bounded(d_empty, (uint32_t)((it - 1) & 1));
        tc_fence_after();
      }
      for (int ch = 0; ch < nchunks; ++ch, ++gch) {
        const int buf = gch % NS, nbuf = (gch + 1) % NS;
        const uint32_t ph = (uint32_t)((gch / NS) & 1);
        if (!ok_a) mbar_wait_bounded(&a_full[buf], ph);
        if (!ok_w) mbar_wait_bounded(&w_full[buf], ph);
        const uint32_t ph1 = (uint32_t)(((gch + 1) / NS) & 1);
        if (!MIX) {
          ok_a = __shfl_sync(0xffffffffu, mbar_test_wait(&a_full[nbuf], ph1) ? 1 : 0, 0);
          ok_w = __shfl_sync(0xffffffffu, mbar_test_wait(&w_full[nbuf], ph1) ? 1 : 0, 0);
        }
        tc_fence_after();
        if (MIX) {
          uint32_t pa = 0, pw = 0;
          if (elect_one_sync()) {
            const uint32_t b_hi = smem_u32(wst) + (uint32_t)(buf * WS_STRIDE);
            mix_mma_chunk_probed<NT>(tmem_d, tmem_d + A_BASE + (uint32_t)(buf * A_STRIDE), umma_smem_desc(b_hi, NT * 16, 128), IDESC, IDESC_BF,
                                 ch != 0 ? 1u : 0u, smem_u32(&a_empty[buf]), smem_u32(&a_full[nbuf]), smem_u32(&w_full[nbuf]),
                                 ph1, pa, pw);
          }
          ok_a = __any_sync(0xffffffffu, pa != 0) ? 1 : 0;
          ok_w = __any_sync(0xffffffffu, pw != 0) ? 1 : 0;
          continue;
        }
        if (elect_one_sync()) {
          const uint32_t b_hi = smem_u32(wst) + (uint32_t)(buf * WS_STRIDE), b_lo = b_hi + tc_b_bytes(NT);
          const uint32_t a_hi = tmem_d + A_BASE + (uint32_t)(buf * A_STRIDE), a_lo = a_hi + 32;
          if (BF16) {
#pragma unroll
            for (int t = 0; t < CT; ++t)
#pragma unroll
              for (int j = 0; j < TC_KC / 16; ++j) {
                const uint64_t db = umma_smem_desc(b_hi + t * W_TAP + j * 2 * (NT * 16), NT * 16, 128);
                umma_ts_f16(tmem_d, a_hi + t * 16 + j * 8, db, IDESC, (ch | t | j) != 0 ? 1u : 0u);
              }
          } else if (MIX) {
            mix_mma_chunk<NT>(tmem_d, a_hi, b_hi, IDESC, IDESC_BF, ch == 0);
          } else {
#pragma unroll
            for (int j = 0; j < TC_KC / 8; ++j) {
              const uint64_t dbh = umma_smem_desc(b_hi + j * 2 * (NT * 16), NT * 16, 128);
              const uint64_t dbl = umma_smem_desc(b_lo + j * 2 * (NT * 16), NT * 16, 128);
              umma_ts_tf32(tmem_d + 64, a_lo + j * 8, dbh, IDESC, (ch | j) != 0 ? 1u : 0u);
              umma_ts_tf32(tmem_d + 64, a_hi + j * 8, dbl, IDESC, 1u);
              umma_ts_tf32(tmem_d, a_hi + j * 8, dbh, IDESC, (ch | j) != 0 ? 1u : 0u);
            }
          }
          umma_commit(&a_empty[buf]);
        }
        __syncwarp();
      }
    }
  } else if (warp == TC_PRODUCERS / 32 + 1) {
    const int ngroups = ncc * NG;
    long long nloads = 0;
    for (int tile = blockIdx.x; tile < ntiles; tile += gridDim.x) nloads += ngroups;
    int l_tile = blockIdx.x, l_cc = 0, l_grp = 0, l_idx = 0;
    auto issue_next_tile = [&]() {
      if (l_idx >= nloads) return;
      if (l_idx >= ntb_rt) mbar_wait_bounded(&t_empty[l_idx % ntb_rt], (uint32_t)(((l_idx / ntb_rt) - 1) & 1));
      if (elect_one_sync()) issue_tile(l_tile, l_cc, l_grp, l_idx);
      __syncwarp();
      ++l_idx;
      if (++l_grp == NG) { l_grp = 0; if (++l_cc == ncc) { l_cc = 0; l_tile += gridDim.x; } }
    };
    for (int i = 0; i < ntb_rt - 1; ++i) issue_next_tile();
    int gch = 0;
    for (int tile = blockIdx.x; tile < ntiles; tile += gridDim.x)
      for (int cc = 0; cc < ncc; ++cc)
        for (int grp = 0; grp < NG; ++grp) {
          issue_next_tile();
          for (int tg = 0; tg < TG; tg += CT, ++gch) {
            const int buf = gch % NS;
            if (gch >= NS) mbar_wait_bounded(&a_empty[buf], (uint32_t)(((gch / NS) - 1) & 1));
            if (elect_one_sync()) {
              mbar_arrive_expect_tx(&w_full[buf], W_BYTES);
#pragma unroll
              for (int t = 0; t < CT; ++t)
                bulk_g2s(wst + buf * WS_STRIDE + t * W_TAP, wimg + (size_t)((grp * TG + tg + t) * ncc + cc) * W_TAP, W_TAP, &w_full[buf],
                         policy_evict_last());
            }
            __syncwarp();
          }
        }
  } else {
    const int row = (warp & 3) * 32 + lane;
    const int kh = warp >> 2;
    const int pr = row / g.TW, pc = row - pr * g.TW;
    const uint32_t lane_addr = tmem_d + ((uint32_t)((warp & 3) * 32) << 16);
    int gch = 0, gcc = 0;
    for (int tile = blockIdx.x; tile < ntiles; tile += gridDim.x) {
      const int img = tile / g.TPI;
      const int trem = tile - img * g.TPI;
      const int tyy = trem / g.TX;
      const int oy0 = tyy * g.TH, ox0 = (trem - tyy * g.TX) * g.TW;
      for (int cc = 0; cc < ncc; ++cc)
      for (int grp = 0; grp < NG; ++grp, ++gcc) {
        const int tb = gcc % ntb_rt;
        int s = 0, c0 = cc * TC_KC;
        if (c0 >= a.src[0].C) { c0 -= a.src[0].C; s = 1; if (c0 >= a.src[1].C) { s = 2; } }
        const bool up = (s == 0 ? a.src[0].uh : (s == 1 ? a.src[1].uh : a.src[2].uh)) == 2;
        const int by = up ? ((oy0 - a.pad) >> 1) : (oy0 - a.pad), bx = up ? ((ox0 - 2 * XH) >> 1) : (S * ox0 - XH);
        const uint32_t esz = SBF ? 2u : 4u;
        const uint32_t cstride = esz * (uint32_t)CHS;
        const uint32_t tile_b = smem_u32(tiles + tb * tile_stride);
        const uint32_t tile_a = tile_b + (uint32_t)(kh * 16) * cstride;
        mbar_wait_bounded(&t_full[tb], (uint32_t)((gcc / ntb_rt) & 1));
#pragma unroll 1
        for (int tg = 0; tg < TG; tg += CT, ++gch) {
          const int buf = gch % NS;
          if constexpr (CT == 3) {
            uint32_t pk[3][8];
#pragma unroll
            for (int t = 0; t < 3; ++t) {
              const int tap = grp * TG + tg + t;
              const int dy = tap / KS, dx = tap - dy * KS;
              int iy = oy0 + pr + dy - a.pad, ix = S * (ox0 + pc) + dx - a.pad;
              const bool zero = a.zi && up && ((iy | ix) & 1);
              if (up) { iy >>= 1; ix >>= 1; }
              const uint32_t qa = tile_a + esz * (uint32_t)((S == 2 ? pr : iy - by) * g.BW + (ix - bx));
              if (SBF) {
                const uint32_t r = (uint32_t)((S == 2 ? pr : iy - by) * g.BW + (ix - bx));
                const uint32_t sw = (r >> 1) & 3u;
#pragma unroll
                for (int q = 0; q < 2; ++q) {
                  const uint32_t ad = tile_b + r * 64u + ((((uint32_t)(kh * 2 + q)) ^ sw) << 4);
                  asm volatile("ld.shared.v4.u32 {%0, %1, %2, %3}, [%4];"
                               : "=r"(pk[t][4 * q]), "=r"(pk[t][4 * q + 1]), "=r"(pk[t][4 * q + 2]), "=r"(pk[t][4 * q + 3]) : "r"(ad));
                }
              } else {
                float v[16];
#pragma unroll
                for (int i = 0; i < 16; ++i) asm volatile("ld.shared.f32 %0, [%1];" : "=f"(v[i]) : "r"(qa + (uint32_t)i * cstride));
#pragma unroll
                for (int i = 0; i < 8; ++i) {
                  const __nv_bfloat162 h2 = __floats2bfloat162_rn(zero ? 0.f : v[2 * i], zero ? 0.f : v[2 * i + 1]);
                  pk[t][i] = *reinterpret_cast<const uint32_t*>(&h2);
                }
              }
            }
            if (gch >= NS) {
              mbar_wait_bounded(&a_empty[buf], (uint32_t)(((gch / NS) - 1) & 1));
              tc_fence_after();
            }
#pragma unroll
            for (int t = 0; t < 3; ++t) tmem_st8(lane_addr + (uint32_t)(A_BASE + buf * A_STRIDE + t * 16 + kh * 8), pk[t]);
            if (tg + CT >= TG) {
              __syncwarp();
              if (lane == 0) mbar_arrive(&t_empty[tb]);
            }
            tmem_st_wait();
            tc_fence_before();
            __syncwarp();
            if (lane == 0) mbar_arrive(&a_full[buf]);
            continue;
          }
          const int tap = grp * TG + tg;
          const int dy = tap / KS, dx = tap - dy * KS;
          int iy = oy0 + pr + dy - a.pad, ix = S * (ox0 + pc) + dx - a.pad;
          const bool zero = a.zi && up && ((iy | ix) & 1);
          if (up) { iy >>= 1; ix >>= 1; }
          const uint32_t qa = tile_a + 4u * (uint32_t)((S == 2 ? pr : iy - by) * g.BW + (ix - bx));
          float v[16];
#pragma unroll
          for (int i = 0; i < 16; ++i) asm volatile("ld.shared.f32 %0, [%1];" : "=f"(v[i]) : "r"(qa + (uint32_t)i * cstride));
          if (zero) {
#pragma unroll
            for (int i = 0; i < 16; ++i) v[i] = 0.f;
          }
          float mhi[16];
          uint32_t mlo2[8], ma2[8];
          if (MIX) mix_split(v, mhi, mlo2, ma2);
          if (gch >= NS) {
            mbar_wait_bounded(&a_empty[buf], (uint32_t)(((gch / NS) - 1) & 1));
            tc_fence_after();
          }
          if (BF16) {
            uint32_t pk[8];
#pragma unroll
            for (int i = 0; i < 8; ++i) {
              const __nv_bfloat162 h2 = __floats2bfloat162_rn(v[2 * i], v[2 * i + 1]);
              pk[i] = *reinterpret_cast<const uint32_t*>(&h2);
            }
            tmem_st8(lane_addr + (uint32_t)(A_BASE + buf * A_STRIDE + kh * 8), pk);
          } else if (MIX) {
            const uint32_t sa = lane_addr + (uint32_t)(A_BASE + buf * A_STRIDE);
            tmem_st16(sa + (uint32_t)(kh * 16), mhi);
            tmem_st8(sa + (uint32_t)(32 + kh * 8), mlo2);
            tmem_st8(sa + (uint32_t)(48 + kh * 8), ma2);
          } else {
            float hi[16], lo[16];
#pragma unroll
            for (int i = 0; i < 16; ++i) {
              hi[i] = __uint_as_float(__float_as_uint(v[i]) & 0xFFFFE000u);
              lo[i] = v[i] - hi[i];
            }
            const uint32_t col = (uint32_t)(A_BASE + buf * A_STRIDE + kh * 16);
            tmem_st16(lane_addr + col, hi);
            tmem_st16(lane_addr + col + 32, lo);
          }
          if (tg == TG - 1) {
            __syncwarp();
            if (lane == 0) mbar_arrive(&t_empty[tb]);
          }
          tmem_st_wait();
          tc_fence_before();
          __syncwarp();
          if (lane == 0) mbar_arrive(&a_full[buf]);
        }
      }
      const int last = gch - 1;
      mbar_wait_bounded(&a_empty[last % NS], (uint32_t)((last / NS) & 1));
      tc_fence_after();

      const int wq = warp & 3, half = warp >> 2;
      const int oy = oy0 + pr, ox = ox0 + pc;
      const bool relu = a.act == CONV_ACT_RELU;
#pragma unroll 1
      for (int pass = 0; pass < NT / 32; ++pass) {
        const int cb = half * (NT / 2) + pass * 16;
        if (cb >= a.Cout) break;
        float acc[16], part[16];
        const uint32_t taddr = tmem_d + ((uint32_t)(wq * 32) << 16) + (uint32_t)cb;
        tmem_ld_cols<16>(taddr, acc);
        if (BF16) {
#pragma unroll
          for (int j = 0; j < 16; ++j) part[j] = 0.f;
        } else {
          tmem_ld_cols<16>(taddr + 64, part);
        }
        const float4* b4 = reinterpret_cast<const float4*>(bias_s + cb);
#pragma unroll
        for (int j = 0; j < 16; j += 4) {
          const float4 bs = b4[j >> 2];
          acc[j] += part[j] + bs.x; acc[j + 1] += part[j + 1] + bs.y; acc[j + 2] += part[j + 2] + bs.z; acc[j + 3] += part[j + 3] + bs.w;
        }
        if (a.skip != nullptr && a.skip_pre) {
          const float* sk = a.skip + ((size_t)img * (a.out_cstride ? a.out_cstride : a.Cout) + cb) * HoWo + (size_t)oy * a.Wo + ox;
#pragma unroll
          for (int j = 0; j < 16; ++j) acc[j] += __ldg(sk + (size_t)j * HoWo);
        }
        if (relu) {
#pragma unroll
          for (int j = 0; j < 16; ++j) acc[j] = fmaxf(acc[j], 0.f);
        } else {
#pragma unroll
          for (int j = 0; j < 16; ++j) acc[j] = tc_act(acc[j], a.act, a.act_scale);
        }
        const size_t o0 = ((size_t)img * (a.out_cstride ? a.out_cstride : a.Cout) + cb) * HoWo + (size_t)oy * a.Wo + ox;
        if (a.skip != nullptr && !a.skip_pre) {
          if (BF16 && a.skip_bf16) {
            const uint4* sk = reinterpret_cast<const uint4*>(reinterpret_cast<const __nv_bfloat16*>(a.skip) +
                                                             (((size_t)img * a.Ho + oy) * a.Wo + ox) * 64 + cb);
#pragma unroll
            for (int q = 0; q < 2; ++q) {
              const uint4 u = __ldg(sk + q);
              const uint32_t w4[4] = {u.x, u.y, u.z, u.w};
#pragma unroll
              for (int i = 0; i < 4; ++i) {
                acc[8 * q + 2 * i] += __uint_as_float(w4[i] << 16);
                acc[8 * q + 2 * i + 1] += __uint_as_float(w4[i] & 0xFFFF0000u);
              }
            }
          } else {
            const float* sk = a.skip + o0;
#pragma unroll
            for (int j = 0; j < 16; ++j) acc[j] += __ldg(sk + (size_t)j * HoWo);
          }
        }
        if (BF16 && a.out_bf16) {
          uint4* po = reinterpret_cast<uint4*>(reinterpret_cast<__nv_bfloat16*>(a.out) + (((size_t)img * a.Ho + oy) * a.Wo + ox) * 64 + cb);
#pragma unroll
          for (int q = 0; q < 2; ++q) {
            uint32_t w4[4];
#pragma unroll
            for (int i = 0; i < 4; ++i) {
              const __nv_bfloat162 h2 = __floats2bfloat162_rn(acc[8 * q + 2 * i], acc[8 * q + 2 * i + 1]);
              w4[i] = *reinterpret_cast<const uint32_t*>(&h2);
            }
            po[q] = make_uint4(w4[0], w4[1], w4[2], w4[3]);
          }
          continue;
        }
        float* po = a.out + o0;
#pragma unroll
        for (int j = 0; j < 16; ++j) po[(size_t)j * HoWo] = acc[j];
      }
      tc_fence_before();
      __syncwarp();
      if (lane == 0) mbar_arrive(d_empty);
    }
  }
  tc_fence_before();
  __syncthreads();
  if (warp == 0) tmem_dealloc(tmem_d, 256);
}


typedef CUresult (*tmap_encode_fn)(CUtensorMap*, CUtensorMapDataType, cuuint32_t, void*, const cuuint64_t*, const cuuint64_t*,
                                   const cuuint32_t*, const cuuint32_t*, CUtensorMapInterleave, CUtensorMapSwizzle,
                                   CUtensorMapL2promotion, CUtensorMapFloatOOBfill);
static tmap_encode_fn tmap_encoder() {
  static const tmap_encode_fn fn = []() -> tmap_encode_fn {
    void* p = nullptr;
    cudaDriverEntryPointQueryResult q;
    if (cudaGetDriverEntryPoint("cuTensorMapEncodeTiled", &p, cudaEnableDefault, &q) == cudaSuccess &&
        q == cudaDriverEntryPointSuccess)
      return reinterpret_cast<tmap_encode_fn>(p);
    return nullptr;
  }();
  return fn;
}

struct TmapKey {
  const void* ptr;
  cuuint64_t dims[4], strides[3];
  cuuint32_t box[4], es[4];
  int rank, swizzle, bf16;
};
static bool tmap_cached(CUtensorMap* out, int rank, const void* ptr, const cuuint64_t* dims, const cuuint64_t* strides,
                        const cuuint32_t* box, const cuuint32_t* es, CUtensorMapSwizzle swz, bool bf16 = false) {
  constexpr int CAP = 96;
  struct Entry { TmapKey k; CUtensorMap m; };
  static thread_local Entry cache[CAP];
  static thread_local int used = 0, next = 0;
  TmapKey k;
  memset(&k, 0, sizeof(k));
  k.ptr = ptr; k.rank = rank; k.swizzle = (int)swz; k.bf16 = bf16 ? 1 : 0;
  for (int i = 0; i < rank; ++i) { k.dims[i] = dims[i]; k.box[i] = box[i]; k.es[i] = es[i]; }
  for (int i = 0; i + 1 < rank; ++i) k.strides[i] = strides[i];
  for (int i = 0; i < used; ++i)
    if (memcmp(&cache[i].k, &k, sizeof(k)) == 0) { *out = cache[i].m; return true; }
  tmap_encode_fn enc = tmap_encoder();
  if (enc == nullptr) return false;
  CUtensorMap m;
  if (enc(&m, bf16 ? CU_TENSOR_MAP_DATA_TYPE_BFLOAT16 : CU_TENSOR_MAP_DATA_TYPE_FLOAT32, (cuuint32_t)rank, const_cast<void*>(ptr), dims, strides, box, es,
          CU_TENSOR_MAP_INTERLEAVE_NONE, swz, CU_TENSOR_MAP_L2_PROMOTION_L2_128B, CU_TENSOR_MAP_FLOAT_OOB_FILL_NONE) != CUDA_SUCCESS)
    return false;
  const int slot = used < CAP ? used++ : (next++ % CAP);
  cache[slot].k = k; cache[slot].m = m;
  *out = m;
  return true;
}

static bool conv_tma_plan(int KS, const ConvArgs& a, ConvTmaArgs* g, int mode = CM_TF32X3) {
  const bool sbf = a.src[0].bf16 != 0;
  if ((sbf || a.out_bf16 || a.skip_bf16) && !(KS == 3 && mode == CM_BF16 && a.Cout == 64)) return false;
  const int XH = KS == 3 ? (sbf ? 1 : TM_XH) : 0;
  if (a.sh != a.sw || (a.sh != 1 && !(a.sh == 2 && KS == 3)) || a.out_nhwc || a.wimg_stride != 0 || (a.Cout != 64 && a.Cout != 32)) return false;
  if (a.pad != (KS == 3 ? 1 : 0)) return false;
  const int S = a.sh;
  const int TWmax = KS == 3 ? 64 : 128;
  const int TW = a.Wo < TWmax ? a.Wo : TWmax;
  if (TW < 16 || 128 % TW || a.Wo % TW) return false;
  const int TH = 128 / TW;
  if (a.Ho % TH) return false;
  const int BW = KS == 3 ? S * TW + 2 * XH : TW, BH = (KS == 3 && S == 1) ? TH + 2 : TH;
  if (BW > 256 || BH > 256 || (size_t)BW * BH * TC_KC * (sbf ? 2 : 4) > (size_t)(sbf ? TM_TILE_BF : tm_tile_bytes(KS))) return false;
  if ((a.out_bf16 || a.skip_bf16) && a.Cout != 64) return false;
  for (int s = 0; s < 3; ++s) {
    const ConvSrc& sc = a.src[s];
    if (sc.C == 0) continue;
    if (sc.nhwc || sc.C % TC_KC || sc.uh != sc.uw || (sc.uh != 1 && sc.uh != 2) || (S == 2 && sc.uh != 1)) return false;
    if ((sc.bf16 != 0) != sbf || (sbf && (sc.uh != 1 || sc.C != 64))) return false;
    if (sc.H * sc.uh != a.Ho * S || sc.W * sc.uw != a.Wo * S) return false;
    if (sbf) {
      if ((uintptr_t)sc.ptr & 15) return false;
      const cuuint64_t dims[4] = {(cuuint64_t)sc.C, (cuuint64_t)sc.W, (cuuint64_t)sc.H, (cuuint64_t)a.B};
      const cuuint64_t strides[3] = {(cuuint64_t)sc.C * 2, (cuuint64_t)sc.W * sc.C * 2, (cuuint64_t)sc.W * sc.H * sc.C * 2};
      const cuuint32_t box[4] = {(cuuint32_t)TC_KC, (cuuint32_t)BW, (cuuint32_t)(BH * S), 1};
      const cuuint32_t es[4] = {1, 1, (cuuint32_t)S, 1};
      if (!tmap_cached(&g->tmap[s], 4, sc.ptr, dims, strides, box, es, CU_TENSOR_MAP_SWIZZLE_64B, true)) return false;
      continue;
    }
    if ((sc.W * 4) % 16 || ((uintptr_t)sc.ptr & 15)) return false;
    const cuuint64_t dims[4] = {(cuuint64_t)sc.W, (cuuint64_t)sc.H, (cuuint64_t)sc.C, (cuuint64_t)a.B};
    const cuuint64_t strides[3] = {(cuuint64_t)sc.W * 4, (cuuint64_t)sc.W * sc.H * 4, (cuuint64_t)sc.W * sc.H * sc.C * 4};
    const cuuint32_t box[4] = {(cuuint32_t)BW, (cuuint32_t)(BH * S), (cuuint32_t)TC_KC, 1};
// ... 1185 lines not shown
  static thread_local int mf_dev = -1;
  int dev = 0;
  TPSPP_CHECK_CUDA(cudaGetDevice(&dev));
  if (mf_dev != dev) {
    TPSPP_CHECK_CUDA(cudaFuncSetAttribute(mlp_fused_kernel, cudaFuncAttributeMaxDynamicSharedMemorySize, MF_SMEM));
    mf_dev = dev;
  }
  const long long ntiles = R / TC_TM;
  dim3 grid((unsigned)min(ntiles, (long long)sm_count()));
  launch_k(mlp_fused_kernel, grid, dim3(MF_THREADS), MF_SMEM, st, g);
  count_launch();
  TPSPP_CHECK_CUDA(cudaGetLastError());
  return TPSPP_OK;
}

int run_down_fused(const float* x, const float* o0, const float* o1, const float* w0img, const float* w1img, const float* w2img,
                   const float* wfimg, const float* b0, const float* b1, const float* b2, const float* bf, float* f0, float* f1,
                   float* f2, float* fg, int B, int h, int w, cudaStream_t st, int out_bf16, int fg_bf16) {
  if (w != 64 || h < 1 || B < 1) return 1;
  if ((((uintptr_t)x | (uintptr_t)o0 | (uintptr_t)o1 | (uintptr_t)w0img | (uintptr_t)w1img | (uintptr_t)w2img | (uintptr_t)wfimg) & 15) != 0)
    return 1;
  TPSPP_REQUIRE(tmap_encoder() != nullptr, "down_fused: cuTensorMapEncodeTiled is not available from this CUDA driver");
  DownFusedArgs g;
  {
    const cuuint64_t dims[4] = {128, (cuuint64_t)(2 * h), 32, (cuuint64_t)B};
    const cuuint64_t strides[3] = {128 * 4, (cuuint64_t)128 * 2 * h * 4, (cuuint64_t)128 * 2 * h * 32 * 4};
    const cuuint32_t box[4] = {64, 2, 32, 1};
    const cuuint32_t es[4] = {1, 1, 1, 1};
    if (!tmap_cached(&g.tm_o0, 4, o0, dims, strides, box, es, CU_TENSOR_MAP_SWIZZLE_NONE)) return 1;
    if (!tmap_cached(&g.tm_o1, 4, o1, dims, strides, box, es, CU_TENSOR_MAP_SWIZZLE_NONE)) return 1;
  }
  {
    const cuuint64_t dims[4] = {64, (cuuint64_t)h, 64, (cuuint64_t)B};
    const cuuint64_t strides[3] = {64 * 4, (cuuint64_t)64 * h * 4, (cuuint64_t)64 * h * 64 * 4};
    const cuuint32_t box[4] = {32, 1, 64, 1};
    const cuuint32_t es[4] = {1, 1, 1, 1};
    if (!tmap_cached(&g.tm_x, 4, x, dims, strides, box, es, CU_TENSOR_MAP_SWIZZLE_NONE)) return 1;
  }
  g.w0img = w0img; g.w1img = w1img; g.w2img = w2img; g.wfimg = wfimg;
  g.b0 = b0; g.b1 = b1; g.b2 = b2; g.bf = bf;
  g.f0 = f0; g.f1 = f1; g.f2 = f2; g.fg = fg; g.B = B; g.h = h; g.out_bf16 = out_bf16; g.fg_bf16 = fg_bf16;
  static thread_local int df_dev = -1;
  int dev = 0;
  TPSPP_CHECK_CUDA(cudaGetDevice(&dev));
  if (df_dev != dev) {
    TPSPP_CHECK_CUDA(cudaFuncSetAttribute(down_fused_kernel, cudaFuncAttributeMaxDynamicSharedMemorySize, DF_SMEM));
    df_dev = dev;
  }
  const long long ntiles = (long long)B * h * 2;
  dim3 grid((unsigned)min(ntiles, (long long)sm_count()));
  launch_k(down_fused_kernel, grid, dim3(DF_THREADS), DF_SMEM, st, g);
  count_launch();
  TPSPP_CHECK_CUDA(cudaGetLastError());
  return TPSPP_OK;
}

int run_score_fused(const float* de2, const float* w0img, const float* w1img, const float* p1img, const float* b0, const float* b1,
                    float* score, int B, int h, int w, int F, float scale, cudaStream_t st) {
  if (w != 64 || F != 32 || h < 2 || (h & 1) || B < 1) return 1;
  if ((((uintptr_t)de2 | (uintptr_t)w0img | (uintptr_t)w1img | (uintptr_t)p1img | (uintptr_t)score) & 15) != 0) return 1;
  TPSPP_REQUIRE(tmap_encoder() != nullptr, "score_fused: cuTensorMapEncodeTiled is not available from this CUDA driver");
  ScoreFusedArgs g;
  const cuuint64_t dims[4] = {64, (cuuint64_t)h, 64, (cuuint64_t)B};
  const cuuint64_t strides[3] = {64 * 4, (cuuint64_t)64 * h * 4, (cuuint64_t)64 * h * 64 * 4};
  const cuuint32_t box[4] = {64, 2, 32, 1};
  const cuuint32_t es[4] = {1, 1, 1, 1};
  if (!tmap_cached(&g.tm_de, 4, de2, dims, strides, box, es, CU_TENSOR_MAP_SWIZZLE_NONE)) return 1;
  g.w0img = w0img; g.w1img = w1img; g.p1img = p1img; g.b0 = b0; g.b1 = b1; g.score = score; g.B = B; g.h = h; g.scale = scale;
  static thread_local int sf_dev = -1;
  int dev = 0;
  TPSPP_CHECK_CUDA(cudaGetDevice(&dev));
  if (sf_dev != dev) {
    TPSPP_CHECK_CUDA(cudaFuncSetAttribute(score_fused_kernel, cudaFuncAttributeMaxDynamicSharedMemorySize, SF_SMEM));
    sf_dev = dev;
  }
  const long long ntiles = (long long)B * (h / 2);
  dim3 grid((unsigned)min(ntiles, (long long)sm_count()));
  launch_k(score_fused_kernel, grid, dim3(SF_THREADS), SF_SMEM, st, g);
  count_launch();
  TPSPP_CHECK_CUDA(cudaGetLastError());
  return TPSPP_OK;
}

int run_conv_tc(int KS, const ConvArgs& a, const float* wprep, int NT, cudaStream_t st, int mode) {
  const bool bf16 = mode == CM_BF16;
  TPSPP_REQUIRE(NT == 64 || NT == 32, "conv_tc: column tile must be 32 or 64");
  TPSPP_REQUIRE(a.Cout % NT == 0 || (NT == 64 && a.Cout == 32), "conv_tc: Cout %d is not a multiple of the column tile %d", a.Cout, NT);
  TPSPP_REQUIRE(KS == 1 || NT == 64 || (a.Cout == 32 && mode == CM_MIX && !a.out_nhwc),
                "conv_tc: 3x3 kernels with a 32-column tile exist for the 32-channel NCHW layers in the mixed operand mode only");
  TPSPP_REQUIRE(tmap_encoder() != nullptr, "conv_tc: cuTensorMapEncodeTiled is not available from this CUDA driver");
  ConvTcArgs t;
  t.c = a;
  t.wprep = wprep;
  const long long M = (long long)a.B * a.Ho * a.Wo;
  dim3 grid((unsigned)((M + TC_TM - 1) / TC_TM), (unsigned)((a.Cout + NT - 1) / NT));
  const bool nhwc = a.src[0].nhwc != 0;
  if (!nhwc && a.wimg_stride == 0 && ((NT == 64 && (a.Cout == 64 || a.Cout == 32)) || (NT == 32 && a.Cout == 32 && !a.out_nhwc))) {
    int dev = 0;
    TPSPP_CHECK_CUDA(cudaGetDevice(&dev));
    ConvTmaArgs g;
    if (conv_tma_plan(KS, a, &g, mode)) {
      g.t = t;
      static thread_local int tma_dev = -1;
      if (tma_dev != dev) {
        TPSPP_CHECK_CUDA(cudaFuncSetAttribute(conv_tma_kernel<1, CM_TF32X3>, cudaFuncAttributeMaxDynamicSharedMemorySize, tm_smem_bytes(1)));
        TPSPP_CHECK_CUDA(cudaFuncSetAttribute(conv_tma_kernel<3, CM_TF32X3>, cudaFuncAttributeMaxDynamicSharedMemorySize, tm_smem_bytes(3)));
        TPSPP_CHECK_CUDA(cudaFuncSetAttribute(conv_tma_kernel<1, CM_BF16>, cudaFuncAttributeMaxDynamicSharedMemorySize, tm_smem_bytes(1)));
        TPSPP_CHECK_CUDA(cudaFuncSetAttribute(conv_tma_kernel<3, CM_BF16>, cudaFuncAttributeMaxDynamicSharedMemorySize, tm_smem_bytes(3)));
        TPSPP_CHECK_CUDA(cudaFuncSetAttribute(conv_tma_kernel<1, CM_MIX>, cudaFuncAttributeMaxDynamicSharedMemorySize, tm_smem_bytes(1)));
        TPSPP_CHECK_CUDA(cudaFuncSetAttribute(conv_tma_kernel<3, CM_MIX>, cudaFuncAttributeMaxDynamicSharedMemorySize, tm_smem_bytes(3)));
        TPSPP_CHECK_CUDA(cudaFuncSetAttribute(conv_tma_kernel<1, CM_TF32X3, 32>, cudaFuncAttributeMaxDynamicSharedMemorySize, tm_smem_bytes(1)));
        TPSPP_CHECK_CUDA(cudaFuncSetAttribute(conv_tma_kernel<3, CM_MIX, 32>, cudaFuncAttributeMaxDynamicSharedMemorySize, tm_smem_bytes(3)));
        tma_dev = dev;
      }
      dim3 pgrid((unsigned)min((long long)grid.x, 2LL * sm_count()));
      if (NT == 32) {
        TPSPP_REQUIRE((KS == 1 && mode == CM_TF32X3) || (KS == 3 && mode == CM_MIX), "conv_tc: the 32-column tile exists for 1x1/3xTF32 and 3x3/mixed only");
        if (KS == 1) launch_k(conv_tma_kernel<1, CM_TF32X3, 32>, pgrid, dim3(TM_THREADS), tm_smem_bytes(1), st, g);
        else launch_k(conv_tma_kernel<3, CM_MIX, 32>, pgrid, dim3(TM_THREADS), tm_smem_bytes(3), st, g);
        count_launch();
        TPSPP_CHECK_CUDA(cudaGetLastError());
        return TPSPP_OK;
      }
      auto kern = KS == 1 ? (mode == CM_BF16 ? conv_tma_kernel<1, CM_BF16> : mode == CM_MIX ? conv_tma_kernel<1, CM_MIX> : conv_tma_kernel<1, CM_TF32X3>)
                          : (mode == CM_BF16 ? conv_tma_kernel<3, CM_BF16> : mode == CM_MIX ? conv_tma_kernel<3, CM_MIX> : conv_tma_kernel<3, CM_TF32X3>);
      launch_k(kern, pgrid, dim3(TM_THREADS), tm_smem_bytes(KS), st, g);
      count_launch();
      TPSPP_CHECK_CUDA(cudaGetLastError());
      return TPSPP_OK;
    }
    TPSPP_REQUIRE(NT == 64, "conv_tc: the 32-column convolution tile needs a TMA-stageable geometry");
    TPSPP_REQUIRE(!a.src[0].bf16 && !a.out_bf16 && !a.skip_bf16, "conv_tc: bf16-stored activations need the TMA-staged 3x3 bf16 kernel");
    static thread_local int ts_dev = -1;
    if (ts_dev != dev) {
      TPSPP_CHECK_CUDA(cudaFuncSetAttribute(conv_ts_kernel<1, CM_TF32X3>, cudaFuncAttributeMaxDynamicSharedMemorySize, TS_SMEM));
      TPSPP_CHECK_CUDA(cudaFuncSetAttribute(conv_ts_kernel<3, CM_TF32X3>, cudaFuncAttributeMaxDynamicSharedMemorySize, TS_SMEM));
      TPSPP_CHECK_CUDA(cudaFuncSetAttribute(conv_ts_kernel<1, CM_BF16>, cudaFuncAttributeMaxDynamicSharedMemorySize, TS_SMEM));
      TPSPP_CHECK_CUDA(cudaFuncSetAttribute(conv_ts_kernel<3, CM_BF16>, cudaFuncAttributeMaxDynamicSharedMemorySize, TS_SMEM));
      TPSPP_CHECK_CUDA(cudaFuncSetAttribute(conv_ts_kernel<1, CM_MIX>, cudaFuncAttributeMaxDynamicSharedMemorySize, TS_SMEM));
      TPSPP_CHECK_CUDA(cudaFuncSetAttribute(conv_ts_kernel<3, CM_MIX>, cudaFuncAttributeMaxDynamicSharedMemorySize, TS_SMEM));
      ts_dev = dev;
    }
    auto kern = KS == 1 ? (mode == CM_BF16 ? conv_ts_kernel<1, CM_BF16> : mode == CM_MIX ? conv_ts_kernel<1, CM_MIX> : conv_ts_kernel<1, CM_TF32X3>)
                        : (mode == CM_BF16 ? conv_ts_kernel<3, CM_BF16> : mode == CM_MIX ? conv_ts_kernel<3, CM_MIX> : conv_ts_kernel<3, CM_TF32X3>);
    launch_k(kern, grid, dim3(TC_THREADS), TS_SMEM, st, t);
    count_launch();
    TPSPP_CHECK_CUDA(cudaGetLastError());
    return TPSPP_OK;
  }
  TPSPP_REQUIRE(mode == CM_TF32X3, "conv_tc: the bf16 / mixed operand modes exist for the NCHW-source convolutions only");
  LinTmaArgs lg;
  const bool lin_ok = KS == 1 && nhwc && lin_tma_plan(a, NT, &lg);
  TPSPP_REQUIRE(a.splitk <= 1 || lin_ok, "conv_tc: split-K exists for the TMA-fed row-major linear kernel only");
  if (lin_ok) {
    lg.t = t;
    int dev = 0;
    TPSPP_CHECK_CUDA(cudaGetDevice(&dev));
    static thread_local int lin_dev = -1;
    if (lin_dev != dev) {
      TPSPP_CHECK_CUDA(cudaFuncSetAttribute(lin_tma_kernel<64>, cudaFuncAttributeMaxDynamicSharedMemorySize, ln_smem_bytes()));
      TPSPP_CHECK_CUDA(cudaFuncSetAttribute(lin_tma_kernel<32>, cudaFuncAttributeMaxDynamicSharedMemorySize, ln_smem_bytes()));
      lin_dev = dev;
    }
    dim3 pgrid((unsigned)min((long long)grid.x, 2LL * sm_count()), lg.col_split ? (unsigned)(a.Cout / NT) : 1u);
    if (lg.col_split) pgrid.x = (unsigned)min((long long)grid.x, max(1LL, 2LL * sm_count() / pgrid.y));
    if (a.splitk > 1) pgrid.z = (unsigned)a.splitk;
    if (NT == 64) launch_k(lin_tma_kernel<64>, pgrid, dim3(TC_THREADS), ln_smem_bytes(), st, lg);
    else launch_k(lin_tma_kernel<32>, pgrid, dim3(TC_THREADS), ln_smem_bytes(), st, lg);
    count_launch();
    TPSPP_CHECK_CUDA(cudaGetLastError());
    return TPSPP_OK;
  }
  if (KS == 3) return nhwc ? launch_tc<3, true, 64>(t, grid, st) : launch_tc<3, false, 64>(t, grid, st);
  if (NT == 64) return nhwc ? launch_tc<1, true, 64>(t, grid, st) : launch_tc<1, false, 64>(t, grid, st);
  return nhwc ? launch_tc<1, true, 32>(t, grid, st) : launch_tc<1, false, 32>(t, grid, st);
}

}
```

### tps_pp_b200/csrc/stage.cu

```cuda
#include "head.cuh"

#include <string.h>

namespace tpspp {

struct FoldItem {
  const float *conv_bias, *gamma, *beta, *mean, *var;
  float *scale, *bias;
  int C;
};
constexpr int STAGE_CONVS = 16;
struct FoldArgs { FoldItem it[STAGE_CONVS]; };
__global__ void __launch_bounds__(64) bnfold_kernel(FoldArgs a) {
  const FoldItem f = a.it[blockIdx.x];
  const int n = threadIdx.x;
  if (n >= f.C) return;
  const double s = (double)__ldg(f.gamma + n) / sqrt((double)__ldg(f.var + n) + 1e-5);
  const double cb = f.conv_bias != nullptr ? (double)__ldg(f.conv_bias + n) : 0.0;
  f.scale[n] = (float)s;
  f.bias[n] = (float)((double)__ldg(f.beta + n) + (cb - (double)__ldg(f.mean + n)) * s);
}

struct StemArgs {
  const float *img, *w, *scale, *bias;
// ... 95 lines not shown

using namespace tpspp;

extern "C" size_t tpspp_stage_workspace_bytes(const tpspp_stage_cfg* cfg) {
  StageDims d;
  if (stage_dims(cfg, &d) != TPSPP_OK) return 0;
  size_t off[SW_COUNT], total;
  stage_offsets(d, off, &total);
  return total;
}

extern "C" int tpspp_stage_fwd(const tpspp_stage_cfg* cfg, const float* img, const float* const* P, float* o0, float* o1,
                               float* x, void* workspace, tpspp_stream_t stream) {
  reset_launch_count();
  prof_begin((cudaStream_t)stream);
  StageDims d;
  int rc = stage_dims(cfg, &d);
  if (rc != TPSPP_OK) return rc;
  if (d.B == 0) return TPSPP_OK;
  TPSPP_REQUIRE(img && P && o0 && o1 && x && workspace, "tpspp_stage_fwd: null pointer");
  TPSPP_REQUIRE(((uintptr_t)workspace & 255) == 0, "tpspp_stage_fwd: workspace must be 256-byte aligned");
  TPSPP_REQUIRE((((uintptr_t)img | (uintptr_t)o0 | (uintptr_t)o1 | (uintptr_t)x) & 15) == 0,
                "tpspp_stage_fwd: image and output buffers must be 16-byte aligned");
  for (int i = 0; i < TPSPP_SP_COUNT; ++i) {
    TPSPP_REQUIRE(P[i] != nullptr, "tpspp_stage_fwd: params[%d] is NULL", i);
    TPSPP_REQUIRE(((uintptr_t)P[i] & 3) == 0, "tpspp_stage_fwd: params[%d] is not a float pointer", i);
  }
  cudaStream_t st = (cudaStream_t)stream;
  struct PdlScope { PdlScope() { pdl_scope(true); } ~PdlScope() { pdl_scope(false); } } pdl_guard;
  size_t off[SW_COUNT], total;
  stage_offsets(d, off, &total);
  auto W = [&](int i) { return reinterpret_cast<float*>((char*)workspace + off[i]); };
  float* fold = W(SW_FOLD);
  const float* wp[STAGE_CONVS - 1];
  {
    float* cur = W(SW_WPREP);
    for (int i = 0; i < STAGE_CONVS - 1; ++i) {
      wp[i] = cur;
      cur += conv_tc_wprep_floats(kStage[i].Cin, kStage[i].KS, kStage[i].Cout);
    }
  }
  if (!(cfg->flags & TPSPP_HEAD_FLAG_WEIGHTS_CACHED)) {
    FoldArgs fa;
    memset(&fa, 0, sizeof(fa));
    fa.it[0] = FoldItem{P[TPSPP_SP_CONV1_B], P[TPSPP_SP_BN1_W], P[TPSPP_SP_BN1_B], P[TPSPP_SP_BN1_MEAN], P[TPSPP_SP_BN1_VAR],
                        fold, fold + 64, 32};
    for (int i = 0; i < STAGE_CONVS - 1; ++i) {
      const int w = kStage[i].w_idx;
      fa.it[i + 1] = FoldItem{nullptr, P[w + 1], P[w + 2], P[w + 3], P[w + 4], fold + 128 * (i + 1), fold + 128 * (i + 1) + 64,
                              kStage[i].Cout};
    }
    bnfold_kernel<<<STAGE_CONVS, 64, 0, st>>>(fa);
    count_launch();
    TPSPP_CHECK_CUDA(cudaGetLastError());
    WPrepLayer L[STAGE_CONVS - 1];
    for (int i = 0; i < STAGE_CONVS - 1; ++i) {
      L[i].w = P[kStage[i].w_idx]; L[i].out = const_cast<float*>(wp[i]); L[i].Ctot = kStage[i].Cin;
      L[i].taps = kStage[i].KS * kStage[i].KS; L[i].N = kStage[i].Cout; L[i].NT = kStage[i].Cout;
      L[i].bf16 = kStage[i].KS == 3 ? CM_MIX : CM_TF32X3;
      L[i].scale = fold + 128 * (i + 1); L[i].dg_cin = 0; L[i].dg_ci0 = 0;
    }
    rc = conv_tc_prepare_weights(L, STAGE_CONVS - 1, st);
    if (rc != TPSPP_OK) return rc;
  }
  {
    StemArgs sa{img, P[TPSPP_SP_CONV1_W], fold, fold + 64, o0, d.B, d.H, d.W};
    const long long total_px = (long long)d.B * d.H * d.W;
    long long blocks = (total_px + 255) / 256;
    if (blocks > 8LL * sm_count()) blocks = 8LL * sm_count();
    launch_k(stem_kernel, dim3((unsigned)blocks), dim3(256), 0, st, sa);
    count_launch();
    TPSPP_CHECK_CUDA(cudaGetLastError());
  }
  auto conv = [&](int i, const float* src, int Hin, int Win, const float* identity, float* out, bool relu) -> int {
    const StageConv& c = kStage[i];
    ConvArgs a;
    memset(&a, 0, sizeof(a));
    a.src[0].ptr = src; a.src[0].C = c.Cin; a.src[0].H = Hin; a.src[0].W = Win; a.src[0].uh = 1; a.src[0].uw = 1; a.src[0].nhwc = 0;
    a.src[1].H = a.src[1].W = a.src[1].uh = a.src[1].uw = 1; a.src[2] = a.src[1];
    a.weight = P[c.w_idx]; a.bias = fold + 128 * (i + 1) + 64; a.skip = identity; a.skip_pre = 1; a.out = out;
    a.B = d.B; a.Ho = Hin / c.stride; a.Wo = Win / c.stride; a.Ctot = c.Cin; a.sh = c.stride; a.sw = c.stride;
    a.pad = c.KS == 3 ? 1 : 0; a.out_nhwc = 0; a.act = relu ? CONV_ACT_RELU : CONV_ACT_NONE; a.act_scale = 1.f;
    a.Cout = c.Cout; a.wimg_stride = 0;
    return run_conv_tc(c.KS, a, wp[i], c.Cout, st, c.KS == 3 ? CM_MIX : CM_TF32X3);
  };
#define CONV(...) do { rc = conv(__VA_ARGS__); if (rc != TPSPP_OK) return rc; } while (0)
  const int H = d.H, Wd = d.W, h = d.h, w = d.w;
  CONV(0, o0, H, Wd, nullptr, W(SW_T1), true);        CONV(1, W(SW_T1), H, Wd, o0, W(SW_YA), true);
  CONV(2, W(SW_YA), H, Wd, nullptr, W(SW_T1), true);  CONV(3, W(SW_T1), H, Wd, W(SW_YA), W(SW_YB), true);
  CONV(4, W(SW_YB), H, Wd, nullptr, W(SW_T1), true);  CONV(5, W(SW_T1), H, Wd, W(SW_YB), o1, true);
  CONV(6, o1, H, Wd, nullptr, W(SW_T2), true);
  CONV(8, o1, H, Wd, nullptr, W(SW_IDN), false);
  CONV(7, W(SW_T2), H, Wd, W(SW_IDN), W(SW_ZA), true);
  CONV(9, W(SW_ZA), h, w, nullptr, W(SW_T3), true);   CONV(10, W(SW_T3), h, w, W(SW_ZA), W(SW_ZB), true);
  CONV(11, W(SW_ZB), h, w, nullptr, W(SW_T3), true);  CONV(12, W(SW_T3), h, w, W(SW_ZB), W(SW_ZA), true);
  CONV(13, W(SW_ZA), h, w, nullptr, W(SW_T3), true);  CONV(14, W(SW_T3), h, w, W(SW_ZA), x, true);
#undef CONV
  return TPSPP_OK;
}
```

### tps_pp_b200/csrc/tc.cuh

```cuda
#pragma once
#include "common.cuh"

namespace tpspp {
#ifdef __CUDACC__

__device__ __forceinline__ uint64_t umma_smem_desc(uint32_t smem_addr, uint32_t lbo_bytes, uint32_t sbo_bytes) {
  uint64_t d = 0;
  d |= (uint64_t)((smem_addr >> 4) & 0x3FFFu);
  d |= (uint64_t)((lbo_bytes >> 4) & 0x3FFFu) << 16;
  d |= (uint64_t)((sbo_bytes >> 4) & 0x3FFFu) << 32;
  d |= (uint64_t)1 << 46;
  return d;
}

__host__ __device__ constexpr uint32_t umma_instr_desc(int M, int N, int fmt) {
  return (1u << 4)
         | ((uint32_t)fmt << 7)
         | ((uint32_t)fmt << 10)
         | ((uint32_t)(N >> 3) << 17)
         | ((uint32_t)(M >> 4) << 24);
}

__device__ __forceinline__ void tmem_alloc(uint32_t* smem_slot, uint32_t ncols) {
  asm volatile("tcgen05.alloc.cta_group::1.sync.aligned.shared::cta.b32 [%0], %1;" ::"r"(smem_u32(smem_slot)),
               "r"(ncols)
               : "memory");
  asm volatile("tcgen05.relinquish_alloc_permit.cta_group::1.sync.aligned;" ::: "memory");
}
__device__ __forceinline__ void tmem_dealloc(uint32_t taddr, uint32_t ncols) {
  asm volatile("tcgen05.dealloc.cta_group::1.sync.aligned.b32 %0, %1;" ::"r"(taddr), "r"(ncols) : "memory");
}
__device__ __forceinline__ void tc_fence_before() { asm volatile("tcgen05.fence::before_thread_sync;" ::: "memory"); }
__device__ __forceinline__ void tc_fence_after() { asm volatile("tcgen05.fence::after_thread_sync;" ::: "memory"); }

template <int KIND>
__device__ __forceinline__ void umma(uint32_t tmem_d, uint64_t adesc, uint64_t bdesc, uint32_t idesc, uint32_t accumulate) {
  if (KIND == 2) {
    asm volatile(
        "{\n.reg .pred p;\nsetp.ne.b32 p, %4, 0;\n"
        "tcgen05.mma.cta_group::1.kind::tf32 [%0], %1, %2, %3, p;\n}\n" ::"r"(tmem_d),
        "l"(adesc), "l"(bdesc), "r"(idesc), "r"(accumulate)
        : "memory");
  } else {
    asm volatile(
        "{\n.reg .pred p;\nsetp.ne.b32 p, %4, 0;\n"
        "tcgen05.mma.cta_group::1.kind::f16 [%0], %1, %2, %3, p;\n}\n" ::"r"(tmem_d),
        "l"(adesc), "l"(bdesc), "r"(idesc), "r"(accumulate)
        : "memory");
  }
}
__device__ __forceinline__ void umma_ts_tf32(uint32_t tmem_d, uint32_t tmem_a, uint64_t bdesc, uint32_t idesc,
                                             uint32_t accumulate) {
  asm volatile(
      "{\n.reg .pred p;\nsetp.ne.b32 p, %4, 0;\n"
      "tcgen05.mma.cta_group::1.kind::tf32 [%0], [%1], %2, %3, p;\n}\n" ::"r"(tmem_d),
      "r"(tmem_a), "l"(bdesc), "r"(idesc), "r"(accumulate)
      : "memory");
}
__device__ __forceinline__ void tmem_st16(uint32_t taddr, const float* v) {
  asm volatile(
      "tcgen05.st.sync.aligned.32x32b.x16.b32 [%0], "
      "{%1, %2, %3, %4, %5, %6, %7, %8, %9, %10, %11, %12, %13, %14, %15, %16};\n" ::"r"(taddr),
      "r"(__float_as_uint(v[0])), "r"(__float_as_uint(v[1])), "r"(__float_as_uint(v[2])), "r"(__float_as_uint(v[3])),
      "r"(__float_as_uint(v[4])), "r"(__float_as_uint(v[5])), "r"(__float_as_uint(v[6])), "r"(__float_as_uint(v[7])),
      "r"(__float_as_uint(v[8])), "r"(__float_as_uint(v[9])), "r"(__float_as_uint(v[10])), "r"(__float_as_uint(v[11])),
      "r"(__float_as_uint(v[12])), "r"(__float_as_uint(v[13])), "r"(__float_as_uint(v[14])), "r"(__float_as_uint(v[15]))
      : "memory");
}
__device__ __forceinline__ void tmem_st8(uint32_t taddr, const uint32_t* v) {
  asm volatile(
      "tcgen05.st.sync.aligned.32x32b.x8.b32 [%0], {%1, %2, %3, %4, %5, %6, %7, %8};\n" ::"r"(taddr),
      "r"(v[0]), "r"(v[1]), "r"(v[2]), "r"(v[3]), "r"(v[4]), "r"(v[5]), "r"(v[6]), "r"(v[7])
      : "memory");
}
__device__ __forceinline__ void umma_ts_f16(uint32_t tmem_d, uint32_t tmem_a, uint64_t bdesc, uint32_t idesc,
                                            uint32_t accumulate) {
  asm volatile(
      "{\n.reg .pred p;\nsetp.ne.b32 p, %4, 0;\n"
      "tcgen05.mma.cta_group::1.kind::f16 [%0], [%1], %2, %3, p;\n}\n" ::"r"(tmem_d),
      "r"(tmem_a), "l"(bdesc), "r"(idesc), "r"(accumulate)
      : "memory");
}
__device__ __forceinline__ void tmem_st_wait() { asm volatile("tcgen05.wait::st.sync.aligned;" ::: "memory"); }

__device__ __forceinline__ void umma_commit(uint64_t* bar) {
  asm volatile("tcgen05.commit.cta_group::1.mbarrier::arrive::one.shared::cluster.b64 [%0];" ::"r"(smem_u32(bar))
               : "memory");
}
__device__ __forceinline__ void tmem_ld32(uint32_t taddr, float* v) {
  uint32_t r[32];
  asm volatile(
      "tcgen05.ld.sync.aligned.32x32b.x32.b32 "
      "{%0, %1, %2, %3, %4, %5, %6, %7, %8, %9, %10, %11, %12, %13, %14, %15, "
      "%16, %17, %18, %19, %20, %21, %22, %23, %24, %25, %26, %27, %28, %29, %30, %31}, [%32];\n"
      : "=r"(r[0]), "=r"(r[1]), "=r"(r[2]), "=r"(r[3]), "=r"(r[4]), "=r"(r[5]), "=r"(r[6]), "=r"(r[7]), "=r"(r[8]),
        "=r"(r[9]), "=r"(r[10]), "=r"(r[11]), "=r"(r[12]), "=r"(r[13]), "=r"(r[14]), "=r"(r[15]), "=r"(r[16]),
        "=r"(r[17]), "=r"(r[18]), "=r"(r[19]), "=r"(r[20]), "=r"(r[21]), "=r"(r[22]), "=r"(r[23]), "=r"(r[24]),
        "=r"(r[25]), "=r"(r[26]), "=r"(r[27]), "=r"(r[28]), "=r"(r[29]), "=r"(r[30]), "=r"(r[31])
      : "r"(taddr)
      : "memory");
  asm volatile("tcgen05.wait::ld.sync.aligned;" ::: "memory");
#pragma unroll
  for (int i = 0; i < 32; ++i) v[i] = __uint_as_float(r[i]);
}

template <int N>
__device__ __forceinline__ void tmem_ld_cols(uint32_t taddr, float* v) {
  if constexpr (N == 32) {
    tmem_ld32(taddr, v);
  } else {
    static_assert(N == 16, "16 or 32 columns");
    uint32_t r[16];
    asm volatile(
// ... 36 lines not shown
```

### tps_pp_b200/functional.py

```python
from __future__ import annotations

import ctypes
from typing import Optional, Tuple

import numpy as np
import torch

from . import _native as N

_DT = {torch.float32: N.F32, torch.bfloat16: N.BF16}
BWD_VARIANT = N.VARIANT_AUTO


def _ptr(t: Optional[torch.Tensor]):
    return None if t is None else ctypes.c_void_p(t.data_ptr())


def _stream(t: torch.Tensor):
    return ctypes.c_void_p(torch.cuda.current_stream(t.device).cuda_stream)


def _require_cuda(name: str, t: Optional[torch.Tensor], dtype=None):
    if t is None:
        return
# ... 130 lines not shown
    return (out0, out1) if src1 is not None else out0


def head_cfg(batch, height, width, point_size, p_stride, precision=N.HEAD_FP32, flags=0) -> N.HeadCfg:
    return N.HeadCfg(int(batch), int(height), int(width), int(point_size[0]), int(point_size[1]), int(p_stride),
                     int(precision), int(flags))


def head_param_shapes(h: int, w: int, f: int, c: int = 64):
    conv3 = lambda ci, co: [(co, ci, 3, 3), (co,)]
    lin = lambda ci, co: [(co, ci), (co,)]
    shapes = conv3(3 * c, 64) + conv3(64, 64) * 3
    shapes += [(64 // 16, 64, 1, 1), (64, 64 // 16, 1, 1), (1, 2, 3, 3), (1,)]
    shapes += conv3(64, 64) * 3 + conv3(64, c)
    shapes += lin(c, 32) + lin(32, 128) + lin(c, 32) + lin(32, 128)
    shapes += [(h, w), (h, w), (h + 1, h + f), (w + 1, w + f)] + lin(c, c) + [(h, w), (h, w)]
    shapes += lin(c, 4 * c) + lin(4 * c, c)
    shapes += lin(c, 256) + lin(256, 2) + lin(2 * f, 2 * f)
    shapes += [(c, 32, 1, 1), (c,)] * 2 + [(c, 64, 1, 1), (c,)] + conv3(c, c) * 2 + [(c, 3 * c, 1, 1), (c,)]
    return shapes


def head_workspace_offsets(cfg: N.HeadCfg):
    arr = (ctypes.c_size_t * len(N.WS_NAMES))()
    N.check(N.lib().tpspp_head_workspace_offsets(ctypes.byref(cfg), arr), "tpspp_head_workspace_offsets")
    return dict(zip(N.WS_NAMES, [int(v) for v in arr]))


def head_forward(x: torch.Tensor, o0: torch.Tensor, o1: torch.Tensor, params, point_size, p_stride,
                 precision=N.HEAD_FP32, workspace: Optional[torch.Tensor] = None, weights_cached: bool = False,
                 flags: int = 0):
    for nm, t in (("batch_img", x), ("outs[0]", o0), ("outs[1]", o1)):
        _require_cuda(nm, t, torch.float32)
    x = x.contiguous(); o0 = o0.contiguous(); o1 = o1.contiguous()
    b, c, h, w = x.shape
    if c != 64 or o0.shape != (b, 32, 2 * h, 2 * w) or o1.shape != (b, 32, 2 * h, 2 * w):
        raise RuntimeError(f"tps_pp_b200: TPS_PP expects batch_img [B,64,h,w] and outs 2x[B,32,2h,2w]; got "
                           f"{tuple(x.shape)}, {tuple(o0.shape)}, {tuple(o1.shape)}")
    params = list(params)
    if len(params) != N.P_COUNT:
        raise RuntimeError(f"tps_pp_b200: expected {N.P_COUNT} parameter tensors, got {len(params)}")
    f = point_size[0] * point_size[1]
    table = (ctypes.c_void_p * N.P_COUNT)()
    for i, (p, shp) in enumerate(zip(params, head_param_shapes(h, w, f))):
        _require_cuda(f"param[{i}]", p, torch.float32)
        if not p.is_contiguous():
            raise RuntimeError(f"tps_pp_b200: param[{i}] must be contiguous")
        if tuple(p.shape) != shp:
            raise RuntimeError(f"tps_pp_b200: param[{i}] has shape {tuple(p.shape)} but a [{b},{c},{h},{w}] input with "
                               f"{f} control points needs {shp} (module built for another img_size / point_size?)")
        table[i] = p.data_ptr()
    cfg = head_cfg(b, h, w, point_size, p_stride, precision, flags)
    with torch.cuda.device(x.device):
        nbytes = int(N.lib().tpspp_head_workspace_bytes(ctypes.byref(cfg)))
        if nbytes == 0 and b > 0:
            raise RuntimeError("tpspp_head_workspace_bytes failed: " + N.last_error())
        if workspace is None or workspace.numel() < nbytes or workspace.device != x.device:
            workspace = torch.empty(max(nbytes, 256), dtype=torch.uint8, device=x.device)
            weights_cached = False
        if weights_cached:
            cfg.flags |= N.HEAD_FLAG_WEIGHTS_CACHED
        fg_bf16 = precision == N.HEAD_BF16 and (flags & N.HEAD_FLAG_FEATGRID_BF16) != 0
        feat_grid = torch.empty((b, 64, 2 * h, 2 * w), dtype=torch.bfloat16 if fg_bf16 else torch.float32, device=x.device)
        c_prime = torch.empty((b, f, 2), dtype=torch.float32, device=x.device)
        score = torch.empty((b, h * w, f), dtype=torch.float32, device=x.device)
        N.check(N.lib().tpspp_head_fwd(ctypes.byref(cfg), _ptr(x), _ptr(o0), _ptr(o1), table, _ptr(feat_grid),
                                       _ptr(c_prime), _ptr(score), _ptr(workspace), _stream(x)), "tpspp_head_fwd")
    return feat_grid, c_prime, score, workspace


def stage_param_shapes():
    def bn(c):
        return [(c,)] * 4
    shapes = [(32, 3, 3, 3), (32,)] + bn(32)
    for cin, planes, blocks, down in ((32, 32, 3, False), (32, 64, 4, True)):
        for i in range(blocks):
            ci = cin if i == 0 else planes
            shapes += [(planes, ci, 1, 1)] + bn(planes) + [(planes, planes, 3, 3)] + bn(planes)
            if i == 0 and down:
                shapes += [(planes, ci, 1, 1)] + bn(planes)
    return shapes


def stage_forward(img: torch.Tensor, params, workspace: Optional[torch.Tensor] = None, weights_cached: bool = False):
    _require_cuda("img", img, torch.float32)
    img = img.contiguous()
    b, c, h, w = img.shape
    if c != 3:
        raise RuntimeError(f"tps_pp_b200: the backbone stage takes 3-channel images, got {tuple(img.shape)}")
    params = list(params)
    shapes = stage_param_shapes()
    if len(params) != N.SP_COUNT:
        raise RuntimeError(f"tps_pp_b200: expected {N.SP_COUNT} stage tensors, got {len(params)}")
    table = (ctypes.c_void_p * N.SP_COUNT)()
    for i, (p, shp) in enumerate(zip(params, shapes)):
        _require_cuda(f"stage param[{i}]", p, torch.float32)
        if not p.is_contiguous() or tuple(p.shape) != shp:
            raise RuntimeError(f"tps_pp_b200: stage param[{i}] must be a contiguous {shp} tensor, got {tuple(p.shape)}")
        table[i] = p.data_ptr()
    cfg = N.StageCfg(b, h, w, N.HEAD_TC, 0)
    with torch.cuda.device(img.device):
        nbytes = int(N.lib().tpspp_stage_workspace_bytes(ctypes.byref(cfg)))
        if nbytes == 0 and b > 0:
            raise RuntimeError("tpspp_stage_workspace_bytes failed: " + N.last_error())
        if workspace is None or workspace.numel() < nbytes or workspace.device != img.device:
            workspace = torch.empty(max(nbytes, 256), dtype=torch.uint8, device=img.device)
            weights_cached = False
        if weights_cached:
            cfg.flags |= N.HEAD_FLAG_WEIGHTS_CACHED
        o0 = torch.empty((b, 32, h, w), dtype=torch.float32, device=img.device)
        o1 = torch.empty((b, 32, h, w), dtype=torch.float32, device=img.device)
        x = torch.empty((b, 64, h // 2, w // 2), dtype=torch.float32, device=img.device)
        N.check(N.lib().tpspp_stage_fwd(ctypes.byref(cfg), _ptr(img), table, _ptr(o0), _ptr(o1), _ptr(x), _ptr(workspace),
                                        _stream(img)), "tpspp_stage_fwd")
    return o0, o1, x, workspace


def locnet_param_keys():
    keys = []
    for ci in (0, 4, 8, 12):
        keys.append(f"conv.{ci}.weight")
        keys += [f"conv.{ci + 1}.{n}" for n in ("weight", "bias", "running_mean", "running_var")]
    return keys + ["localization_fc1.0.weight", "localization_fc1.0.bias", "localization_fc2.weight", "localization_fc2.bias"]


def locnet_param_shapes(channels: int, num_fiducial: int):
    shapes = []
    chans = (channels, 64, 128, 256, 512)
    for i in range(4):
        shapes.append((chans[i + 1], chans[i], 3, 3))
        shapes += [(chans[i + 1],)] * 4
    return shapes + [(256, 512), (256,), (2 * num_fiducial, 256), (2 * num_fiducial,)]


def locnet_supported(channels: int, height: int, width: int, num_fiducial: int) -> bool:
    cfg = N.LocnetCfg(1, channels, height, width, num_fiducial, 0)
    return int(N.lib().tpspp_locnet_workspace_bytes(ctypes.byref(cfg))) > 0


def locnet_forward(img: torch.Tensor, params, num_fiducial: int, workspace: Optional[torch.Tensor] = None,
                   weights_cached: bool = False):
    _require_cuda("img", img, torch.float32)
    if len(params) != N.LP_COUNT:
        raise RuntimeError(f"tps_pp_b200: the localisation network takes {N.LP_COUNT} parameter tensors, got {len(params)}")
    img = img.contiguous()
    b, c, h, w = img.shape
    for i, (t, shp) in enumerate(zip(params, locnet_param_shapes(c, num_fiducial))):
        _require_cuda(f"params[{i}]", t, torch.float32)
        if not t.is_contiguous():
            raise RuntimeError(f"tps_pp_b200: params[{i}] must be contiguous")
        if tuple(t.shape) != shp:
            raise RuntimeError(f"tps_pp_b200: localisation-network params[{i}] has shape {tuple(t.shape)}, expected {shp} for "
                               f"{c} image channels and {num_fiducial} control points")
    cfg = N.LocnetCfg(b, c, h, w, num_fiducial, 0)
    table = (ctypes.c_void_p * N.LP_COUNT)(*[t.data_ptr() for t in params])
    with torch.cuda.device(img.device):
        nbytes = int(N.lib().tpspp_locnet_workspace_bytes(ctypes.byref(cfg)))
        if nbytes == 0 and b > 0:
            raise RuntimeError("tpspp_locnet_workspace_bytes failed: " + N.last_error())
        if workspace is None or workspace.numel() < nbytes or workspace.device != img.device:
            workspace = torch.empty(max(nbytes, 256), dtype=torch.uint8, device=img.device)
            weights_cached = False
        if weights_cached:
            cfg.flags |= N.HEAD_FLAG_WEIGHTS_CACHED
        cp = torch.empty((b, num_fiducial, 2), dtype=torch.float32, device=img.device)
        N.check(N.lib().tpspp_locnet_fwd(ctypes.byref(cfg), _ptr(img), table, _ptr(cp), _ptr(workspace), _stream(img)),
                "tpspp_locnet_fwd")
    return cp, workspace


def _conv_cfg(b, cin, h, w, k, sh, sw, relu, ups):
    cfg = N.ConvCfg(b, cin, h, w, k, sh, sw, 1 if relu else 0, len(ups))
    for i, (uh, uw) in enumerate(ups):
        cfg.up_h[i] = uh
        cfg.up_w[i] = uw
    return cfg


def _ptr_array(ts):
    arr = (ctypes.c_void_p * 3)()
    for i, t in enumerate(ts):
        arr[i] = t.data_ptr() if t is not None else None
    return arr
# ... 309 lines not shown
```

Before: 179,700.

## Run mixed-mode 3x3 convolutions on a CTA pair with cta_group::2 UMMA

Adds a 2-CTA cluster variant of the TMA conv kernel for the 64-column mixed-precision 3x3 path. It uses tcgen05 cta_group::2 MMAs over a 256-row tile, allocates TMEM for the pair, and loads half of the weight tile per CTA through a cluster TMA. Producer arrivals are forwarded to the leader CTA's barriers. The pair path is on by default when the tile count is even; a flag disables it. The aim is to halve per-CTA weight traffic and raise MMA efficiency, at the cost of cross-CTA synchronisation and cluster scheduling limits.

New measurement: 121,300, median of 6. 0.675x the previous value.

```diff
diff --git a/include/tpspp.h b/include/tpspp.h
--- a/include/tpspp.h
+++ b/include/tpspp.h
@@ -96,7 +96,7 @@
 } tpspp_head_cfg;
 
 enum { TPSPP_HEAD_FLAG_WEIGHTS_CACHED = 1, TPSPP_HEAD_FLAG_UNFUSED_DOWN = 2, TPSPP_HEAD_FLAG_UNFUSED_SCORE = 4,
-       TPSPP_HEAD_FLAG_TF32X3_CONV = 8, TPSPP_HEAD_FLAG_FEATGRID_BF16 = 16 };
+       TPSPP_HEAD_FLAG_TF32X3_CONV = 8, TPSPP_HEAD_FLAG_FEATGRID_BF16 = 16, TPSPP_HEAD_FLAG_CONV_SINGLE_CTA = 32 };
 
 enum {
   TPSPP_P_ENC0_W = 0, TPSPP_P_ENC0_B, TPSPP_P_ENC1_W, TPSPP_P_ENC1_B, TPSPP_P_ENC2_W, TPSPP_P_ENC2_B,
diff --git a/tps_pp_b200/_native.py b/tps_pp_b200/_native.py
--- a/tps_pp_b200/_native.py
+++ b/tps_pp_b200/_native.py
@@ -74,6 +74,7 @@
 HEAD_FLAG_UNFUSED_SCORE = 4
 HEAD_FLAG_TF32X3_CONV = 8
 HEAD_FLAG_FEATGRID_BF16 = 16
+HEAD_FLAG_CONV_SINGLE_CTA = 32
 LINEAR_FLAG_WEIGHTS_CACHED = 1
 ACT_NONE, ACT_GELU = 0, 1
 ABI_VERSION = 2
diff --git a/tps_pp_b200/backbone.py b/tps_pp_b200/backbone.py
--- a/tps_pp_b200/backbone.py
+++ b/tps_pp_b200/backbone.py
@@ -68,6 +68,7 @@
             planes *= 2
         self.stage_impl = "auto"
         self._stage_ws = {}
+        self.stage_flags = 0
         self._last_stage_native = None
 
     def init_weights(self):
@@ -110,7 +111,7 @@
             key = (img.device.index, torch.cuda.current_stream(img.device).cuda_stream)
             stamp = (img.shape[0], img.shape[2], tuple((t.data_ptr(), t._version) for t in tensors))
             ws, ws_stamp = self._stage_ws.get(key, (None, None))
-            o0, o1, x, ws = TF.stage_forward(img, tensors, ws, weights_cached=(ws_stamp == stamp))
+            o0, o1, x, ws = TF.stage_forward(img, tensors, ws, weights_cached=(ws_stamp == stamp), flags=self.stage_flags)
             if len(self._stage_ws) >= 8 and key not in self._stage_ws:
                 self._stage_ws.clear()
             self._stage_ws[key] = (ws, stamp)
diff --git a/tps_pp_b200/csrc/common.cuh b/tps_pp_b200/csrc/common.cuh
--- a/tps_pp_b200/csrc/common.cuh
+++ b/tps_pp_b200/csrc/common.cuh
@@ -21,22 +21,36 @@
 bool pdl_on();
 void pdl_scope(bool on);
 template <typename... KArgs, typename... Args>
-inline void launch_k(void (*kern)(KArgs...), dim3 grid, dim3 block, size_t smem, cudaStream_t st, Args&&... args) {
+inline void launch_kc(void (*kern)(KArgs...), dim3 grid, dim3 block, size_t smem, cudaStream_t st, unsigned cluster, Args&&... args) {
   cudaLaunchConfig_t cfg = {};
   cfg.gridDim = grid;
   cfg.blockDim = block;
   cfg.dynamicSmemBytes = smem;
   cfg.stream = st;
-  cudaLaunchAttribute at[1];
-  at[0].id = cudaLaunchAttributeProgrammaticStreamSerialization;
-  at[0].val.programmaticStreamSerializationAllowed = 1;
+  cudaLaunchAttribute at[2];
+  unsigned n = 0;
+  if (cluster > 1) {
+    at[n].id = cudaLaunchAttributeClusterDimension;
+    at[n].val.clusterDim.x = cluster; at[n].val.clusterDim.y = 1; at[n].val.clusterDim.z = 1;
+    ++n;
+  }
+  const unsigned base = n;
+  if (pdl_on()) {
+    at[n].id = cudaLaunchAttributeProgrammaticStreamSerialization;
+    at[n].val.programmaticStreamSerializationAllowed = 1;
+    ++n;
+  }
   cfg.attrs = at;
-  cfg.numAttrs = pdl_on() ? 1 : 0;
-  if (cudaLaunchKernelEx(&cfg, kern, static_cast<KArgs>(args)...) != cudaSuccess && cfg.numAttrs != 0) {
+  cfg.numAttrs = n;
+  if (cudaLaunchKernelEx(&cfg, kern, static_cast<KArgs>(args)...) != cudaSuccess && cfg.numAttrs != base) {
     cudaGetLastError();
-    cfg.numAttrs = 0;
+    cfg.numAttrs = base;
     cudaLaunchKernelEx(&cfg, kern, static_cast<KArgs>(args)...);
   }
+}
+template <typename... KArgs, typename... Args>
+inline void launch_k(void (*kern)(KArgs...), dim3 grid, dim3 block, size_t smem, cudaStream_t st, Args&&... args) {
+  launch_kc(kern, grid, block, smem, st, 1u, static_cast<Args&&>(args)...);
 }
 #ifdef __CUDACC__
 __device__ __forceinline__ void pdl_wait() { asm volatile("griddepcontrol.wait;" ::: "memory"); }
diff --git a/tps_pp_b200/csrc/head.cu b/tps_pp_b200/csrc/head.cu
--- a/tps_pp_b200/csrc/head.cu
+++ b/tps_pp_b200/csrc/head.cu
@@ -826,7 +826,7 @@
   ConvSrc s; s.ptr = p; s.C = C; s.H = H; s.W = W; s.uh = uh; s.uw = uw; s.nhwc = nhwc; s.bf16 = bf16; return s;
 }
 
-static int run_conv(int KS, ConvSrc s0, ConvSrc s1, ConvSrc s2, const float* w, const float* bias, const float* skip,
+static int run_conv(bool pair, int KS, ConvSrc s0, ConvSrc s1, ConvSrc s2, const float* w, const float* bias, const float* skip,
                     float* out, int out_nhwc, int B, int Ho, int Wo, int sh, int sw, cudaStream_t st,
                     const float* wprep = nullptr, int mode = CM_TF32X3, int out_bf16 = 0, int skip_bf16 = 0) {
   ConvArgs a;
@@ -835,7 +835,7 @@
   a.src[0] = s0; a.src[1] = s1; a.src[2] = s2;
   a.weight = w; a.bias = bias; a.skip = skip; a.out = out;
   a.B = B; a.Ho = Ho; a.Wo = Wo; a.Ctot = s0.C + s1.C + s2.C; a.sh = sh; a.sw = sw; a.pad = (KS == 3) ? 1 : 0;
-  if (wprep != nullptr && conv_tc_eligible(a, KS)) return run_conv_tc(KS, a, wprep, 64, st, mode);
+  if (wprep != nullptr && conv_tc_eligible(a, KS)) return run_conv_tc(KS, a, wprep, 64, st, mode, pair);
   const long long M = (long long)B * Ho * Wo;
   const unsigned grid = (unsigned)((M + CV_TM - 1) / CV_TM);
   if (KS == 1) conv_ffma_kernel<1><<<grid, 256, CV_SMEM, st>>>(a);
@@ -933,7 +933,8 @@
       if (rc != TPSPP_OK) return rc;
     }
   }
-#define RUN(...) do { rc = run_conv(__VA_ARGS__); if (rc != TPSPP_OK) return rc; } while (0)
+  const bool pair = !(cfg->flags & TPSPP_HEAD_FLAG_CONV_SINGLE_CTA);
+#define RUN(...) do { rc = run_conv(pair, __VA_ARGS__); if (rc != TPSPP_OK) return rc; } while (0)
   bool fused_down = false;
   if (tc && !(cfg->flags & TPSPP_HEAD_FLAG_UNFUSED_DOWN)) {
     rc = run_down_fused(x, o0, o1, wp[0], wp[1], wp[2], wp[5], P[TPSPP_P_DOWN0_B], P[TPSPP_P_DOWN1_B], P[TPSPP_P_DOWN2_B],
diff --git a/tps_pp_b200/csrc/head.cuh b/tps_pp_b200/csrc/head.cuh
--- a/tps_pp_b200/csrc/head.cuh
+++ b/tps_pp_b200/csrc/head.cuh
@@ -32,7 +32,7 @@
 
 
 bool conv_tc_eligible(const ConvArgs& a, int KS);
-int run_conv_tc(int KS, const ConvArgs& a, const float* wprep, int NT, cudaStream_t st, int mode = CM_TF32X3);
+int run_conv_tc(int KS, const ConvArgs& a, const float* wprep, int NT, cudaStream_t st, int mode = CM_TF32X3, bool pair = false);
 int run_mlp_fused(const float* v, const float* x1, const float* w1img, const float* b1, const float* w2img, const float* b2,
                   float* out, long long R, cudaStream_t st);
 int run_down_fused(const float* x, const float* o0, const float* o1, const float* w0img, const float* w1img, const float* w2img,
diff --git a/tps_pp_b200/csrc/head_tc.cu b/tps_pp_b200/csrc/head_tc.cu
--- a/tps_pp_b200/csrc/head_tc.cu
+++ b/tps_pp_b200/csrc/head_tc.cu
@@ -267,45 +267,59 @@
     umma_ts_tf32(tmem_d, a_base + j * 8, dbh, idesc_tf, (first && j == 0) ? 0u : 1u);
   }
 }
-template <int NT>
+#define TPSPP_MIX_CHUNK_ASM(CG, COMMIT)                                                                \
+  "{\n"                                                                                                \
+  ".reg .pred pa, pw, pf, pt;\n"                                                                       \
+  ".reg .b64 dsc;\n"                                                                                   \
+  ".reg .b32 ta, tc;\n"                                                                                \
+  "mbarrier.test_wait.parity.shared::cta.b64 pa, [%2], %4;\n"                                          \
+  "mbarrier.test_wait.parity.shared::cta.b64 pw, [%3], %4;\n"                                          \
+  "setp.ne.b32 pf, %9, 0;\n"                                                                           \
+  "setp.eq.u32 pt, %4, %4;\n"                                                                          \
+  "add.u32 tc, %5, 64;\n"                                                                              \
+   \
+  "add.u32 ta, %6, 32;\n add.u64 dsc, %7, %12;\n"                                                      \
+  "tcgen05.mma.cta_group::" CG ".kind::f16 [tc], [ta], dsc, %11, pf;\n"                                \
+  "add.u32 ta, %6, 48;\n add.u64 dsc, %7, %13;\n"                                                      \
+  "tcgen05.mma.cta_group::" CG ".kind::f16 [tc], [ta], dsc, %11, pt;\n"                                \
+  "add.u32 ta, %6, 40;\n add.u64 dsc, %7, %14;\n"                                                      \
+  "tcgen05.mma.cta_group::" CG ".kind::f16 [tc], [ta], dsc, %11, pt;\n"                                \
+  "add.u32 ta, %6, 56;\n add.u64 dsc, %7, %15;\n"                                                      \
+  "tcgen05.mma.cta_group::" CG ".kind::f16 [tc], [ta], dsc, %11, pt;\n"                                \
+                                                               \
+  "tcgen05.mma.cta_group::" CG ".kind::tf32 [%5], [%6], %7, %10, pf;\n"                                \
+  "add.u32 ta, %6, 8;\n add.u64 dsc, %7, %16;\n"                                                       \
+  "tcgen05.mma.cta_group::" CG ".kind::tf32 [%5], [ta], dsc, %10, pt;\n"                               \
+  "add.u32 ta, %6, 16;\n add.u64 dsc, %7, %17;\n"                                                      \
+  "tcgen05.mma.cta_group::" CG ".kind::tf32 [%5], [ta], dsc, %10, pt;\n"                               \
+  "add.u32 ta, %6, 24;\n add.u64 dsc, %7, %18;\n"                                                      \
+  "tcgen05.mma.cta_group::" CG ".kind::tf32 [%5], [ta], dsc, %10, pt;\n"                               \
+  COMMIT                                                                                               \
+  "selp.u32 %0, 1, 0, pa;\n"                                                                           \
+  "selp.u32 %1, 1, 0, pw;\n"                                                                           \
+  "}\n"
+template <int NT, int CG = 1>
 __device__ __forceinline__ void mix_mma_chunk_probed(uint32_t d, uint32_t a_base, uint64_t bdesc0, uint32_t idesc_tf, uint32_t idesc_bf,
                                                      uint32_t accumulate, uint32_t commit_bar, uint32_t next_a_bar, uint32_t next_w_bar,
                                                      uint32_t next_parity, uint32_t& ok_a, uint32_t& ok_w) {
+  static_assert(CG == 1 || CG == 2, "cta_group::1 or ::2");
   constexpr int KS2 = 2 * NT, BW0 = 8 * NT, BL0 = 12 * NT;
-  asm volatile(
-      "{\n"
-      ".reg .pred pa, pw, pf, pt;\n"
-      ".reg .b64 dsc;\n"
-      ".reg .b32 ta, tc;\n"
-      "mbarrier.test_wait.parity.shared::cta.b64 pa, [%2], %4;\n"
-      "mbarrier.test_wait.parity.shared::cta.b64 pw, [%3], %4;\n"
-      "setp.ne.b32 pf, %9, 0;\n"
-      "setp.eq.u32 pt, %4, %4;\n"
-      "add.u32 tc, %5, 64;\n"
-      "add.u32 ta, %6, 32;\n add.u64 dsc, %7, %12;\n"
-      "tcgen05.mma.cta_group::1.kind::f16 [tc], [ta], dsc, %11, pf;\n"
-      "add.u32 ta, %6, 48;\n add.u64 dsc, %7, %13;\n"
-      "tcgen05.mma.cta_group::1.kind::f16 [tc], [ta], dsc, %11, pt;\n"
-      "add.u32 ta, %6, 40;\n add.u64 dsc, %7, %14;\n"
-      "tcgen05.mma.cta_group::1.kind::f16 [tc], [ta], dsc, %11, pt;\n"
-      "add.u32 ta, %6, 56;\n add.u64 dsc, %7, %15;\n"
-      "tcgen05.mma.cta_group::1.kind::f16 [tc], [ta], dsc, %11, pt;\n"
-      "tcgen05.mma.cta_group::1.kind::tf32 [%5], [%6], %7, %10, pf;\n"
-      "add.u32 ta, %6, 8;\n add.u64 dsc, %7, %16;\n"
-      "tcgen05.mma.cta_group::1.kind::tf32 [%5], [ta], dsc, %10, pt;\n"
-      "add.u32 ta, %6, 16;\n add.u64 dsc, %7, %17;\n"
-      "tcgen05.mma.cta_group::1.kind::tf32 [%5], [ta], dsc, %10, pt;\n"
-      "add.u32 ta, %6, 24;\n add.u64 dsc, %7, %18;\n"
-      "tcgen05.mma.cta_group::1.kind::tf32 [%5], [ta], dsc, %10, pt;\n"
-      "tcgen05.commit.cta_group::1.mbarrier::arrive::one.shared::cluster.b64 [%8];\n"
-      "selp.u32 %0, 1, 0, pa;\n"
-      "selp.u32 %1, 1, 0, pw;\n"
-      "}\n"
-      : "=r"(ok_a), "=r"(ok_w)
-      : "r"(next_a_bar), "r"(next_w_bar), "r"(next_parity), "r"(d), "r"(a_base), "l"(bdesc0), "r"(commit_bar), "r"(accumulate),
-        "r"(idesc_tf), "r"(idesc_bf), "n"(BW0), "n"(BL0), "n"(BW0 + KS2), "n"(BL0 + KS2), "n"(KS2), "n"(2 * KS2), "n"(3 * KS2)
-      : "memory");
-}
+  if constexpr (CG == 1) {
+    asm volatile(TPSPP_MIX_CHUNK_ASM("1", "tcgen05.commit.cta_group::1.mbarrier::arrive::one.shared::cluster.b64 [%8];\n")
+                 : "=r"(ok_a), "=r"(ok_w)
+                 : "r"(next_a_bar), "r"(next_w_bar), "r"(next_parity), "r"(d), "r"(a_base), "l"(bdesc0), "r"(commit_bar), "r"(accumulate),
+                   "r"(idesc_tf), "r"(idesc_bf), "n"(BW0), "n"(BL0), "n"(BW0 + KS2), "n"(BL0 + KS2), "n"(KS2), "n"(2 * KS2), "n"(3 * KS2)
+                 : "memory");
+  } else {
+    asm volatile(TPSPP_MIX_CHUNK_ASM("2", "tcgen05.commit.cta_group::2.mbarrier::arrive::one.shared::cluster.multicast::cluster.b64 [%8], %19;\n")
+                 : "=r"(ok_a), "=r"(ok_w)
+                 : "r"(next_a_bar), "r"(next_w_bar), "r"(next_parity), "r"(d), "r"(a_base), "l"(bdesc0), "r"(commit_bar), "r"(accumulate),
+                   "r"(idesc_tf), "r"(idesc_bf), "n"(BW0), "n"(BL0), "n"(BW0 + KS2), "n"(BL0 + KS2), "n"(KS2), "n"(2 * KS2), "n"(3 * KS2),
+                   "h"((uint16_t)0x3)
+                 : "memory");
+  }
+}
+#undef TPSPP_MIX_CHUNK_ASM
 __device__ __forceinline__ void mix_split(const float (&v)[16], float (&hi)[16], uint32_t (&lo2)[8], uint32_t (&a2)[8]) {
 #pragma unroll
   for (int i = 0; i < 16; ++i) hi[i] = __uint_as_float(__float_as_uint(v[i]) & 0xFFFFE000u);
@@ -597,6 +611,7 @@
 struct ConvTmaArgs {
   ConvTcArgs t;
   CUtensorMap tmap[3];
+  CUtensorMap wmap;
   int TW, TH, BW, BH;
   int TX, TPI;
   int S;
@@ -619,9 +634,31 @@
       : "memory");
 }
 
-template <int KS, int MODE, int NT = 64>
+__device__ __forceinline__ void tma_load_w_half(void* dst, const CUtensorMap* tm, int c0, int c1, uint32_t bar_cluster, uint64_t policy) {
+  asm volatile(
+      "cp.async.bulk.tensor.2d.cta_group::2.shared::cluster.global.mbarrier::complete_tx::bytes.L2::cache_hint "
+      "[%0], [%1, {%2, %3}], [%4], %5;" ::"r"(smem_u32(dst)),
+      "l"(reinterpret_cast<uint64_t>(tm)), "r"(c0), "r"(c1), "r"(bar_cluster), "l"(policy)
+      : "memory");
+}
+template <bool PAIR>
+__device__ __forceinline__ void tm_wait(uint64_t* bar, uint32_t parity) {
+  if constexpr (PAIR) {
+#pragma unroll 1
+    for (uint32_t it = 0; it < (1u << 28); ++it)
+      if (mbar_try_wait(bar, parity)) return;
+    printf("conv_tma_kernel (CTA pair): mbarrier wait timed out: block %d thread %d barrier smem 0x%x parity %u\n", (int)blockIdx.x,
+           (int)threadIdx.x, smem_u32(bar), parity);
+    __trap();
+  } else {
+    mbar_wait_bounded(bar, parity);
+  }
+}
+
+template <int KS, int MODE, int NT = 64, bool PAIR = false>
 __global__ void __launch_bounds__(TM_THREADS, 2) conv_tma_kernel(const __grid_constant__ ConvTmaArgs g) {
   constexpr bool BF16 = MODE == CM_BF16, MIX = MODE == CM_MIX;
+  static_assert(!PAIR || (KS == 3 && MIX && NT == 64), "the CTA-pair form exists for the 64-column mixed-mode 3x3 kernel");
   constexpr int T = KS * KS;
   static_assert(NT == 64 || NT == 32, "64 or 32 output channels per tile");
   const int XH = g.XH;
@@ -652,18 +689,29 @@
   const ConvArgs& a = g.t.c;
   const int tid = threadIdx.x, lane = tid & 31;
   const int warp = __shfl_sync(0xffffffffu, tid >> 5, 0);
+  const uint32_t rank = PAIR ? cluster_ctarank() : 0u;
+  constexpr int NCTA = PAIR ? 2 : 1;
+  constexpr int NB = NT / NCTA;
 
   if (tid == 0) {
-    for (int i = 0; i < NS; ++i) { mbar_init(&a_empty[i], 1); mbar_init(&a_full[i], TC_PRODUCERS / 32); mbar_init(&w_full[i], 1); }
+    for (int i = 0; i < NS; ++i) { mbar_init(&a_empty[i], 1); mbar_init(&a_full[i], NCTA * TC_PRODUCERS / 32); mbar_init(&w_full[i], 1); }
     for (int i = 0; i < 4; ++i) { mbar_init(&t_full[i], 1); mbar_init(&t_empty[i], TC_PRODUCERS / 32); }
-    mbar_init(d_empty, TC_PRODUCERS / 32);
+    mbar_init(d_empty, NCTA * TC_PRODUCERS / 32);
     fence_barrier_init();
   }
   if (tid < NT) bias_s[tid] = (a.bias != nullptr && tid < a.Cout) ? __ldg(a.bias + tid) : 0.f;
-  if (warp == 0) tmem_alloc(tmem_slot, 256);
+  if (warp == 0) {
+    if (PAIR) tmem_alloc_pair(tmem_slot, 256);
+    else tmem_alloc(tmem_slot, 256);
+  }
   tc_fence_before();
   __syncthreads();
+  if (PAIR) cluster_sync();
   tc_fence_after();
+  auto arrive_leader = [&](uint64_t* bar) {
+    if (PAIR) mbar_arrive_cluster(mapa_shared(bar, 0));
+    else mbar_arrive(bar);
+  };
   const uint32_t tmem_d = *tmem_slot;
   pdl_trigger();
   pdl_wait();
@@ -675,8 +723,8 @@
   const int CHS = g.BW * g.BH;
   const uint32_t tile_tx = (uint32_t)(CHS * TC_KC * (SBF ? 2 : 4));
   const unsigned char* wimg = reinterpret_cast<const unsigned char*>(g.t.wprep);
-  constexpr uint32_t IDESC = umma_instr_desc(TC_TM, NT, BF16 ? 1 : 2);
-  constexpr uint32_t IDESC_BF = umma_instr_desc(TC_TM, NT, 1);
+  constexpr uint32_t IDESC = umma_instr_desc(NCTA * TC_TM, NT, BF16 ? 1 : 2);
+  constexpr uint32_t IDESC_BF = umma_instr_desc(NCTA * TC_TM, NT, 1);
 
   const int S = g.S, NG = (KS == 3 && S == 2) ? 3 : 1, TG = T / NG;
   auto issue_tile = [&](int tile, int cc, int grp, int gcc) {
@@ -700,16 +748,16 @@
   if (warp == TC_PRODUCERS / 32) {
     int gch = 0, it = 0;
     int ok_a = 0, ok_w = 0;
-    for (int tile = blockIdx.x; tile < ntiles; tile += gridDim.x, ++it) {
+    for (int tile = (PAIR && rank != 0) ? ntiles : (int)blockIdx.x; tile < ntiles; tile += gridDim.x, ++it) {
       if (it >= 1) {
-        mbar_wait_bounded(d_empty, (uint32_t)((it - 1) & 1));
+        tm_wait<PAIR>(d_empty, (uint32_t)((it - 1) & 1));
         tc_fence_after();
       }
       for (int ch = 0; ch < nchunks; ++ch, ++gch) {
         const int buf = gch % NS, nbuf = (gch + 1) % NS;
         const uint32_t ph = (uint32_t)((gch / NS) & 1);
-        if (!ok_a) mbar_wait_bounded(&a_full[buf], ph);
-        if (!ok_w) mbar_wait_bounded(&w_full[buf], ph);
+        if (!ok_a) tm_wait<PAIR>(&a_full[buf], ph);
+        if (!ok_w) tm_wait<PAIR>(&w_full[buf], ph);
         const uint32_t ph1 = (uint32_t)(((gch + 1) / NS) & 1);
         if (!MIX) {
           ok_a = __shfl_sync(0xffffffffu, mbar_test_wait(&a_full[nbuf], ph1) ? 1 : 0, 0);
@@ -720,9 +768,9 @@
           uint32_t pa = 0, pw = 0;
           if (elect_one_sync()) {
             const uint32_t b_hi = smem_u32(wst) + (uint32_t)(buf * WS_STRIDE);
-            mix_mma_chunk_probed<NT>(tmem_d, tmem_d + A_BASE + (uint32_t)(buf * A_STRIDE), umma_smem_desc(b_hi, NT * 16, 128), IDESC, IDESC_BF,
-                                 ch != 0 ? 1u : 0u, smem_u32(&a_empty[buf]), smem_u32(&a_full[nbuf]), smem_u32(&w_full[nbuf]),
-                                 ph1, pa, pw);
+            mix_mma_chunk_probed<NB, NCTA>(tmem_d, tmem_d + A_BASE + (uint32_t)(buf * A_STRIDE), umma_smem_desc(b_hi, NB * 16, 128), IDESC,
+                                           IDESC_BF, ch != 0 ? 1u : 0u, smem_u32(&a_empty[buf]), smem_u32(&a_full[nbuf]),
+                                           smem_u32(&w_full[nbuf]), ph1, pa, pw);
           }
           ok_a = __any_sync(0xffffffffu, pa != 0) ? 1 : 0;
           ok_w = __any_sync(0xffffffffu, pw != 0) ? 1 : 0;
@@ -763,7 +811,7 @@
     int l_tile = blockIdx.x, l_cc = 0, l_grp = 0, l_idx = 0;
     auto issue_next_tile = [&]() {
       if (l_idx >= nloads) return;
-      if (l_idx >= ntb_rt) mbar_wait_bounded(&t_empty[l_idx % ntb_rt], (uint32_t)(((l_idx / ntb_rt) - 1) & 1));
+      if (l_idx >= ntb_rt) tm_wait<PAIR>(&t_empty[l_idx % ntb_rt], (uint32_t)(((l_idx / ntb_rt) - 1) & 1));
       if (elect_one_sync()) issue_tile(l_tile, l_cc, l_grp, l_idx);
       __syncwarp();
       ++l_idx;
@@ -777,7 +825,16 @@
           issue_next_tile();
           for (int tg = 0; tg < TG; tg += CT, ++gch) {
             const int buf = gch % NS;
-            if (gch >= NS) mbar_wait_bounded(&a_empty[buf], (uint32_t)(((gch / NS) - 1) & 1));
+            if (gch >= NS) tm_wait<PAIR>(&a_empty[buf], (uint32_t)(((gch / NS) - 1) & 1));
+            if (PAIR) {
+              if (elect_one_sync()) {
+                if (rank == 0) mbar_arrive_expect_tx(&w_full[buf], W_BYTES);
+                tma_load_w_half(wst + buf * WS_STRIDE, &g.wmap, (int)rank * 128, (grp * TG + tg) * ncc * 16 + cc * 16,
+                                mapa_shared(&w_full[buf], 0), policy_evict_last());
+              }
+              __syncwarp();
+              continue;
+            }
             if (elect_one_sync()) {
               mbar_arrive_expect_tx(&w_full[buf], W_BYTES);
 #pragma unroll
@@ -810,7 +867,7 @@
         const uint32_t cstride = esz * (uint32_t)CHS;
         const uint32_t tile_b = smem_u32(tiles + tb * tile_stride);
         const uint32_t tile_a = tile_b + (uint32_t)(kh * 16) * cstride;
-        mbar_wait_bounded(&t_full[tb], (uint32_t)((gcc / ntb_rt) & 1));
+        tm_wait<PAIR>(&t_full[tb], (uint32_t)((gcc / ntb_rt) & 1));
 #pragma unroll 1
         for (int tg = 0; tg < TG; tg += CT, ++gch) {
           const int buf = gch % NS;
@@ -877,7 +934,7 @@
           uint32_t mlo2[8], ma2[8];
           if (MIX) mix_split(v, mhi, mlo2, ma2);
           if (gch >= NS) {
-            mbar_wait_bounded(&a_empty[buf], (uint32_t)(((gch / NS) - 1) & 1));
+            tm_wait<PAIR>(&a_empty[buf], (uint32_t)(((gch / NS) - 1) & 1));
             tc_fence_after();
           }
           if (BF16) {
@@ -911,11 +968,11 @@
           tmem_st_wait();
           tc_fence_before();
           __syncwarp();
-          if (lane == 0) mbar_arrive(&a_full[buf]);
+          if (lane == 0) arrive_leader(&a_full[buf]);
         }
       }
       const int last = gch - 1;
-      mbar_wait_bounded(&a_empty[last % NS], (uint32_t)((last / NS) & 1));
+      tm_wait<PAIR>(&a_empty[last % NS], (uint32_t)((last / NS) & 1));
       tc_fence_after();
 
       const int wq = warp & 3, half = warp >> 2;
@@ -993,12 +1050,18 @@
       }
       tc_fence_before();
       __syncwarp();
-      if (lane == 0) mbar_arrive(d_empty);
+      if (lane == 0) arrive_leader(d_empty);
     }
   }
   tc_fence_before();
   __syncthreads();
-  if (warp == 0) tmem_dealloc(tmem_d, 256);
+  if (PAIR) {
+    cluster_sync();
+    tc_fence_after();
+    if (warp == 0) tmem_dealloc_pair(tmem_d, 256);
+  } else {
+    if (warp == 0) tmem_dealloc(tmem_d, 256);
+  }
 }
 
 
@@ -2350,7 +2413,45 @@
   return TPSPP_OK;
 }
 
-int run_conv_tc(int KS, const ConvArgs& a, const float* wprep, int NT, cudaStream_t st, int mode) {
+static bool conv_pair_wins(const ConvArgs& a, const ConvTmaArgs& g) {
+  const long long ntiles = (long long)a.B * a.Ho * a.Wo / TC_TM;
+  (void)g;
+  return ntiles % 2 == 0;
+}
+
+static int launch_conv_pair(const ConvArgs& a, ConvTmaArgs& g, cudaStream_t st, int dev) {
+  auto kern = conv_tma_kernel<3, CM_MIX, 64, true>;
+  const int nchunks = a.Ctot / TC_KC * 9;
+  const cuuint64_t dims[2] = {256, (cuuint64_t)nchunks * 16};
+  const cuuint64_t strides[1] = {1024};
+  const cuuint32_t box[2] = {128, 16};
+  const cuuint32_t es[2] = {1, 1};
+  TPSPP_REQUIRE(tmap_cached(&g.wmap, 2, g.t.wprep, dims, strides, box, es, CU_TENSOR_MAP_SWIZZLE_NONE),
+                "conv_tc: cannot encode the tensor map of the weight image");
+  static thread_local int pair_dev = -1, pair_clusters = 0;
+  if (pair_dev != dev) {
+    TPSPP_CHECK_CUDA(cudaFuncSetAttribute(kern, cudaFuncAttributeMaxDynamicSharedMemorySize, tm_smem_bytes(3)));
+    cudaLaunchConfig_t cfg = {};
+    cfg.gridDim = dim3(2 * sm_count());
+    cfg.blockDim = dim3(TM_THREADS);
+    cfg.dynamicSmemBytes = tm_smem_bytes(3);
+    cudaLaunchAttribute at[1];
+    at[0].id = cudaLaunchAttributeClusterDimension;
+    at[0].val.clusterDim.x = 2; at[0].val.clusterDim.y = 1; at[0].val.clusterDim.z = 1;
+    cfg.attrs = at;
+    cfg.numAttrs = 1;
+    TPSPP_CHECK_CUDA(cudaOccupancyMaxActiveClusters(&pair_clusters, kern, &cfg));
+    TPSPP_REQUIRE(pair_clusters > 0, "conv_tc: no CTA pair of the 3x3 kernel fits this device");
+    pair_dev = dev;
+  }
+  const long long npairs = min((long long)a.B * a.Ho * a.Wo / TC_TM / 2, (long long)pair_clusters);
+  launch_kc(kern, dim3((unsigned)(2 * npairs)), dim3(TM_THREADS), tm_smem_bytes(3), st, 2u, g);
+  count_launch();
+  TPSPP_CHECK_CUDA(cudaGetLastError());
+  return TPSPP_OK;
+}
+
+int run_conv_tc(int KS, const ConvArgs& a, const float* wprep, int NT, cudaStream_t st, int mode, bool pair) {
   const bool bf16 = mode == CM_BF16;
   TPSPP_REQUIRE(NT == 64 || NT == 32, "conv_tc: column tile must be 32 or 64");
   TPSPP_REQUIRE(a.Cout % NT == 0 || (NT == 64 && a.Cout == 32), "conv_tc: Cout %d is not a multiple of the column tile %d", a.Cout, NT);
@@ -2382,6 +2483,7 @@
         tma_dev = dev;
       }
       dim3 pgrid((unsigned)min((long long)grid.x, 2LL * sm_count()));
+      if (pair && NT == 64 && KS == 3 && mode == CM_MIX && conv_pair_wins(a, g)) return launch_conv_pair(a, g, st, dev);
       if (NT == 32) {
         TPSPP_REQUIRE((KS == 1 && mode == CM_TF32X3) || (KS == 3 && mode == CM_MIX), "conv_tc: the 32-column tile exists for 1x1/3xTF32 and 3x3/mixed only");
         if (KS == 1) launch_k(conv_tma_kernel<1, CM_TF32X3, 32>, pgrid, dim3(TM_THREADS), tm_smem_bytes(1), st, g);
diff --git a/tps_pp_b200/csrc/stage.cu b/tps_pp_b200/csrc/stage.cu
--- a/tps_pp_b200/csrc/stage.cu
+++ b/tps_pp_b200/csrc/stage.cu
@@ -201,7 +201,7 @@
     a.B = d.B; a.Ho = Hin / c.stride; a.Wo = Win / c.stride; a.Ctot = c.Cin; a.sh = c.stride; a.sw = c.stride;
     a.pad = c.KS == 3 ? 1 : 0; a.out_nhwc = 0; a.act = relu ? CONV_ACT_RELU : CONV_ACT_NONE; a.act_scale = 1.f;
     a.Cout = c.Cout; a.wimg_stride = 0;
-    return run_conv_tc(c.KS, a, wp[i], c.Cout, st, c.KS == 3 ? CM_MIX : CM_TF32X3);
+    return run_conv_tc(c.KS, a, wp[i], c.Cout, st, c.KS == 3 ? CM_MIX : CM_TF32X3, !(cfg->flags & TPSPP_HEAD_FLAG_CONV_SINGLE_CTA));
   };
 #define CONV(...) do { rc = conv(__VA_ARGS__); if (rc != TPSPP_OK) return rc; } while (0)
   const int H = d.H, Wd = d.W, h = d.h, w = d.w;
diff --git a/tps_pp_b200/csrc/tc.cuh b/tps_pp_b200/csrc/tc.cuh
--- a/tps_pp_b200/csrc/tc.cuh
+++ b/tps_pp_b200/csrc/tc.cuh
@@ -29,6 +29,31 @@
 }
 __device__ __forceinline__ void tmem_dealloc(uint32_t taddr, uint32_t ncols) {
   asm volatile("tcgen05.dealloc.cta_group::1.sync.aligned.b32 %0, %1;" ::"r"(taddr), "r"(ncols) : "memory");
+}
+__device__ __forceinline__ void tmem_alloc_pair(uint32_t* smem_slot, uint32_t ncols) {
+  asm volatile("tcgen05.alloc.cta_group::2.sync.aligned.shared::cta.b32 [%0], %1;" ::"r"(smem_u32(smem_slot)),
+               "r"(ncols)
+               : "memory");
+  asm volatile("tcgen05.relinquish_alloc_permit.cta_group::2.sync.aligned;" ::: "memory");
+}
+__device__ __forceinline__ void tmem_dealloc_pair(uint32_t taddr, uint32_t ncols) {
+  asm volatile("tcgen05.dealloc.cta_group::2.sync.aligned.b32 %0, %1;" ::"r"(taddr), "r"(ncols) : "memory");
+}
+__device__ __forceinline__ uint32_t cluster_ctarank() {
+  uint32_t r;
+  asm volatile("mov.u32 %0, %%cluster_ctarank;" : "=r"(r));
+  return r;
+}
+__device__ __forceinline__ void cluster_sync() {
+  asm volatile("barrier.cluster.arrive.release.aligned;\nbarrier.cluster.wait.acquire.aligned;" ::: "memory");
+}
+__device__ __forceinline__ uint32_t mapa_shared(const void* p, uint32_t rank) {
+  uint32_t r;
+  asm volatile("mapa.shared::cluster.u32 %0, %1, %2;" : "=r"(r) : "r"(smem_u32(p)), "r"(rank));
+  return r;
+}
+__device__ __forceinline__ void mbar_arrive_cluster(uint32_t cluster_addr) {
+  asm volatile("mbarrier.arrive.shared::cluster.b64 _, [%0];" ::"r"(cluster_addr) : "memory");
 }
 __device__ __forceinline__ void tc_fence_before() { asm volatile("tcgen05.fence::before_thread_sync;" ::: "memory"); }
 __device__ __forceinline__ void tc_fence_after() { asm volatile("tcgen05.fence::after_thread_sync;" ::: "memory"); }
diff --git a/tps_pp_b200/functional.py b/tps_pp_b200/functional.py
--- a/tps_pp_b200/functional.py
+++ b/tps_pp_b200/functional.py
@@ -236,7 +236,8 @@
     return shapes
 
 
-def stage_forward(img: torch.Tensor, params, workspace: Optional[torch.Tensor] = None, weights_cached: bool = False):
+def stage_forward(img: torch.Tensor, params, workspace: Optional[torch.Tensor] = None, weights_cached: bool = False,
+                  flags: int = 0):
     _require_cuda("img", img, torch.float32)
     img = img.contiguous()
     b, c, h, w = img.shape
@@ -252,7 +253,7 @@
         if not p.is_contiguous() or tuple(p.shape) != shp:
             raise RuntimeError(f"tps_pp_b200: stage param[{i}] must be a contiguous {shp} tensor, got {tuple(p.shape)}")
         table[i] = p.data_ptr()
-    cfg = N.StageCfg(b, h, w, N.HEAD_TC, 0)
+    cfg = N.StageCfg(b, h, w, N.HEAD_TC, int(flags))
     with torch.cuda.device(img.device):
         nbytes = int(N.lib().tpspp_stage_workspace_bytes(ctypes.byref(cfg)))
         if nbytes == 0 and b > 0:
```
